# adityaX1412/Experiment-YOLO

Hardware: AMD Instinct MI355X
Metric: images/sec (train) DEAL-YOLO-N 640x640 bs=64/GPU (higher is better)
Workload: dtype f16; 1 GPU; DEAL-YOLO-N (yolov8n-ASF-P2P2.yaml) train step 640x640, per-GPU batch 64, fwd+TAL/WIOU+NWD/DFL/BCE loss+bwd+SGD+EMA, BASELINE.json configs[1]; loss_mode=wiou+nwd, settle_steps=18, capture_retries=0, global_batch=64, parallelism=dp1, hipgraph=True

## Files before the change

experiment-yolo_amd/csrc/conv_wgrad.hip:

```cpp
#include <cstdio>
#include "common.h"
#include "dealyolo_hip.h"

typedef short short4v __attribute__((ext_vector_type(4)));
typedef unsigned int u32x4 __attribute__((ext_vector_type(4)));

struct WgArgs {
  const f16* x;
  const f16* dy;
  float* slabs;
  int ldx, lddy;
  int N, H, W, Ho, Wo;
  int cin_p, cout_p;
  int cin_r8, cout_r8;
  int nci_chunks;
  int tiles_x, tiles_y, ntiles;
  long npix;
  const f16* raw;
  f16* draw;
  const float* coef;
  const double* acc;
  float* dgamma;
  float* dbeta;
  int ldraw, cout;
  float count;
  DySegs xs;
  int dy_csplit;
  unsigned dy_plane;
  const f16* wt;
  f16* dx;
  int lddx, dx_acc;
  int dg_mt, dg_rows;
  DySegs dxs;
};

static __device__ __forceinline__ half8 tr_frag(const char* base0, const char* base1) {
  union {
    short4v s[2];
    half8 h;
  } u;
  u.s[0] = __builtin_amdgcn_ds_read_tr16_b64_v4i16((LDS_AS short4v*)(base0));
  u.s[1] = __builtin_amdgcn_ds_read_tr16_b64_v4i16((LDS_AS short4v*)(base1));
  return u.h;
}

static constexpr __host__ __device__ int wg_th(int ks, int stride, int nci, int mtc) {
  if (ks == 1) return (nci + mtc <= 4) ? 8 : 4;
  if (stride == 1) return (nci * mtc <= 1) ? 16 : ((nci + mtc <= 4) ? 8 : 4);
  return (nci * mtc <= 1) ? 8 : ((nci + mtc <= 4) ? 4 : 2);
}

template <int KS, int STRIDE, int NCI, int MTC, int BNF>
__global__ __launch_bounds__(256, (BNF & 8) ? 3 : ((KS == 3 && NCI * MTC >= 16) ? 1 : 2)) void conv_wgrad_kernel(const WgArgs a) {
  constexpr bool FLAT = (KS == 1);
  constexpr bool DG = (BNF & 4) != 0;
  constexpr bool NOX = (BNF & 8) != 0;
  static_assert(!NOX || DG, "the form without X exists for the fused input gradient only");
  constexpr bool BN1 = ((BNF & 3) == 1 || (BNF & 3) == 3);
  constexpr bool XSEG = ((BNF & 3) == 3);
  static_assert(!DG || (KS == 1 && BN1), "the fused input gradient exists for the 1x1 BatchNorm forms");
  constexpr int TAPS = KS * KS;
  constexpr int NCOL = NCI * TAPS;
  constexpr int CPW = (NCOL + 3) / 4;
  constexpr int TH = wg_th(KS, STRIDE, NCI, MTC), TW = 32;
  constexpr int HWX = FLAT ? TH * TW : (TW - 1) * STRIDE + KS;
  constexpr int HHX = FLAT ? 1 : (TH - 1) * STRIDE + KS;
  constexpr int PAD = KS / 2;
  constexpr int CIN_C = 16 * NCI, COUT_C = 16 * MTC;
  constexpr int PSX = (STRIDE == 2) ? CIN_C * 2 + 16 : (((CIN_C / 2 + 7) / 16) * 16 + 8) * 4;
  constexpr int PSY = (((COUT_C / 2 + 7) / 16) * 16 + 8) * 4;
  constexpr int XBYTES = NOX ? 0 : HHX * HWX * PSX, YBYTES = TH * TW * PSY;
  __shared__ __attribute__((aligned(16))) char smem[XBYTES + YBYTES];
  char* const sx = smem;
  char* const sy = smem + XBYTES;
  __shared__ __attribute__((aligned(16))) float sbn[BN1 ? 4 * COUT_C : (BNF == 2 ? 256 * 8 : 4)];
  float bsum[8] = {0.f, 0.f, 0.f, 0.f, 0.f, 0.f, 0.f, 0.f};
  (void)bsum;
  constexpr int DKS = MTC == 4 ? 2 : (MTC == 3 ? 3 : 1), DCPK = (MTC & 1) ? 16 : 32;
  constexpr int DNT = TH / 2;
  constexpr int DNC = 4 * NCI;
  constexpr int DXROW = CIN_C * 2 + 16;
  constexpr int DPPR = CIN_C / 8;
  constexpr int DPIXPASS = 64 / DPPR > 16 ? 16 : 64 / DPPR;
  constexpr int DNPASS = (16 + DPIXPASS - 1) / DPIXPASS;
  __shared__ __attribute__((aligned(16))) char sdx[DG ? 4 * 16 * DXROW : 16];

  const int tid = threadIdx.x, wave = tid >> 6, lane = tid & 63, p = lane & 15, q = lane >> 4;
  const int qq = p >> 2, pp = p & 3;
  const int co_chunk = blockIdx.y / a.nci_chunks, ci_chunk = blockIdx.y - co_chunk * a.nci_chunks;
  const int ci0 = ci_chunk * CIN_C, co0 = co_chunk * COUT_C;

  f32x4 acc[NOX ? 1 : MTC][NOX ? 1 : CPW];
  if (!NOX) {
#pragma unroll
    for (int m = 0; m < MTC; ++m)
#pragma unroll
      for (int c = 0; c < CPW; ++c) acc[NOX ? 0 : m][NOX ? 0 : c] = (f32x4){0.f, 0.f, 0.f, 0.f};
  }
  (void)acc;

  constexpr int NGX = HHX * HWX * (CIN_C / 8), NGY = TH * TW * (COUT_C / 8);
  constexpr int NPX = NOX ? 1 : (NGX + 255) / 256, NPY = (NGY + 255) / 256;
  uint4 pfx[NPX], pfy[NPY];
  uint4 pfr[BN1 ? NPY : 1];
  unsigned roff[BN1 ? NPY : 1];
  int ncur = 0, nnext = 0;
  (void)ncur; (void)nnext;
  unsigned vnext = 0, vcur = 0, ornext = 0, orcur = 0;
  (void)pfr; (void)roff; (void)vnext; (void)vcur; (void)ornext; (void)orcur;
  constexpr unsigned NEVER = 0x80000000u;
  constexpr int CPGX = CIN_C / 8, CPGY = COUT_C / 8;
  unsigned xoff[NPX], yoff[NPY];
  (void)pfx; (void)xoff;
#pragma unroll
  for (int i = 0; i < NPX; ++i) {
    const int id = tid + i * 256;
    const int pixel = id / CPGX, part = id - pixel * CPGX;
    const bool ok = !NOX && id < NGX && ci0 + part * 8 < a.cin_r8;
    const int hy = FLAT ? 0 : pixel / HWX, hx = FLAT ? pixel : pixel - hy * HWX;
    xoff[i] = ok ? (unsigned)(((hy * a.W + hx) * a.ldx + ci0 + part * 8) * 2) : NEVER;
  }
  constexpr bool XIN = XSEG && !NOX;
  const char* xb[XIN ? NPX : 1];
  int xl[XIN ? NPX : 1];
  unsigned xup = 0;
  bool any_up = false;
  if (XIN)
    for (int k = 0; k < a.xs.nseg; ++k) any_up = any_up || (a.xs.acc[k] & 2);
  (void)xb; (void)xl; (void)xup; (void)any_up;
  if (XIN) {
#pragma unroll
    for (int i = 0; i < NPX; ++i) {
      const int id = tid + i * 256;
      const int part = id % CPGX, ch = ci0 + part * 8;
      int sg = 0;
      while (sg + 1 < a.xs.nseg && ch >= a.xs.c_end[sg]) ++sg;
      const int cb = sg ? a.xs.c_end[sg - 1] : 0;
      const bool ok = id < NGX && ch < a.cin_r8;
      xb[XIN ? i : 0] = ok ? reinterpret_cast<const char*>(a.xs.ptr[sg]) + (ch - cb) * 2 : nullptr;
      xl[XIN ? i : 0] = a.xs.ld[sg] * 2;
      if (ok && (a.xs.acc[sg] & 2)) xup |= 1u << i;
    }
  }
#pragma unroll
  for (int i = 0; i < NPY; ++i) {
    const int id = tid + i * 256;
    const int pixel = id / CPGY, part = id - pixel * CPGY;
    const bool ok = id < NGY && co0 + part * 8 < a.cout_r8;
    const int ty = FLAT ? 0 : pixel / TW, tx = FLAT ? pixel : pixel - ty * TW;
    yoff[i] = ok ? (unsigned)(((ty * a.Wo + tx) * a.lddy + co0 + part * 8) * 2) : NEVER;
    if (FLAT && BN1 && a.dy_csplit && ok) {
      const int ch = co0 + part * 8;
      yoff[i] = (unsigned)((tx * a.lddy + (ch < a.dy_csplit ? ch : ch - a.dy_csplit)) * 2) + (ch < a.dy_csplit ? 0u : a.dy_plane);
    }
    if (BN1) roff[i] = ok ? (unsigned)(((ty * a.Wo + tx) * a.ldraw + co0 + part * 8) * 2) : NEVER;
  }
  if (BN1) {
    for (int c = tid; c < COUT_C; c += 256) {
      const int ch = co0 + c;
      float sc = 0.f, sh = 0.f, kb = 0.f, kc = 0.f;
      if (ch < a.cout) {
        double s1 = 0.0, s2 = 0.0;
#pragma unroll
        for (int k = 0; k < DY_BN_COPIES; ++k) {
          s1 += a.acc[(size_t)(k * 2 + 0) * a.cout + ch];
          s2 += a.acc[(size_t)(k * 2 + 1) * a.cout + ch];
        }
        const float mg = (float)(s1 / a.count), mgx = (float)(s2 / a.count);
        sc = a.coef[ch];
        sh = a.coef[a.cout + ch];
        const float mean = a.coef[2 * a.cout + ch], inv = a.coef[3 * a.cout + ch];
        kb = sc * inv * mgx;
        kc = sc * mg - kb * mean;
        if (!NOX && blockIdx.x == 0 && ci_chunk == 0) {
          if (a.dbeta) a.dbeta[ch] = (float)s1;
          if (a.dgamma) a.dgamma[ch] = (float)s2;
        }
      }
      sbn[c] = sc;
      sbn[COUT_C + c] = sh;
      sbn[2 * COUT_C + c] = kb;
      sbn[3 * COUT_C + c] = kc;
    }
    __syncthreads();
  }
  half8 wf[DG ? DKS : 1][DG ? NCI : 1];
  unsigned dboff[DG ? DKS : 1];
  char* dxb = nullptr;
  unsigned dxld2 = 0;
  bool dxacc = false, dxadd = false;
  const int dpix = lane / DPPR, dpiece = lane - dpix * DPPR;
  (void)wf; (void)dboff; (void)dxb; (void)dxld2; (void)dxacc; (void)dxadd; (void)dpix; (void)dpiece;
  if (DG) {
#pragma unroll
    for (int k = 0; k < DKS; ++k) {
      dboff[DG ? k : 0] = (unsigned)((k * DCPK + ((q * 8) & (DCPK - 1))) * 2);
#pragma unroll
      for (int j = 0; j < NCI; ++j) {
        const int ch = ci0 + (p >> 2) * DNC + 4 * j + (p & 3);
        const int gw = 16 * a.dg_mt, g = ch / gw, rem = ch - g * gw;
        const int row = g * gw + ((rem % (4 * a.dg_mt)) >> 2) * 16 + (rem / (4 * a.dg_mt)) * 4 + (rem & 3);
        const int grow = (g * DKS + k) * gw + (row - g * gw);
        half8 v;
#pragma unroll
        for (int e = 0; e < 8; ++e) v[e] = (f16)0.f;
        if (row < a.dg_rows) v = *reinterpret_cast<const half8*>(a.wt + ((size_t)grow * 32 + q * 8));
        wf[DG ? k : 0][DG ? j : 0] = v;
      }
    }
    const int chn = ci0 + dpiece * 8;
    if (lane < DPIXPASS * DPPR && chn < a.cin_r8) {
      if (XSEG) {
        int sg = 0;
        while (sg + 1 < a.dxs.nseg && chn >= a.dxs.c_end[sg]) ++sg;
        const int cb = sg ? a.dxs.c_end[sg - 1] : 0;
        dxb = reinterpret_cast<char*>(const_cast<void*>(a.dxs.ptr[sg])) + (chn - cb) * 2;
        dxld2 = (unsigned)a.dxs.ld[sg] * 2u;
        dxacc = a.dxs.acc[sg] != 0;
      } else {
        dxb = reinterpret_cast<char*>(a.dx) + chn * 2;
        dxld2 = (unsigned)a.lddx * 2u;
        dxacc = a.dx_acc != 0;
      }
    }
    if (XSEG) {
      for (int k = 0; k < a.dxs.nseg; ++k) dxadd = dxadd || a.dxs.acc[k] != 0;
    } else {
      dxadd = a.dx_acc != 0;
    }
  }
  union DU4 { uint4 u; half2_ h[4]; };
  DU4 dold[DG ? DNT : 1][DG ? DNPASS : 1];
  (void)dold;
  auto ld16 = [](__amdgpu_buffer_rsrc_t r, unsigned off) {
    const auto v = __builtin_amdgcn_raw_buffer_load_b128(r, (int)off, 0, 0);
    return *reinterpret_cast<const uint4*>(&v);
  };
  auto prefetch = [&](int tile) {
    if (FLAT) {
      const auto rx = __builtin_amdgcn_make_buffer_rsrc(const_cast<f16*>(a.x), 0, (int)((unsigned)a.npix * (unsigned)a.ldx * 2u), 0x00020000);
      const auto ry = __builtin_amdgcn_make_buffer_rsrc(const_cast<f16*>(a.dy), 0, (int)((unsigned)a.npix * (unsigned)a.lddy * 2u + (a.dy_csplit ? a.dy_plane : 0u)), 0x00020000);
      const unsigned ox = (unsigned)tile * (TH * TW) * a.ldx * 2u, oy = (unsigned)tile * (TH * TW) * a.lddy * 2u;
      if (NOX) {
      } else if (XIN) {
        const long p0 = (long)tile * (TH * TW);
        int n0 = 0, y0 = 0, x0 = 0;
        if (any_up) {
          const int hw = a.H * a.W, g0 = (int)p0;
          n0 = g0 / hw;
          const int r0 = g0 - n0 * hw;
          y0 = r0 / a.W;
          x0 = r0 - y0 * a.W;
        }
        const float invW = 1.0f / (float)a.W, invH = 1.0f / (float)a.H;
#pragma unroll
        for (int i = 0; i < NPX; ++i) {
          const int lp = (tid + i * 256) / CPGX;
          long gp = p0 + lp;
          const bool inside = gp < a.npix;
          if ((xup >> i) & 1u) {
            const int xx = x0 + lp, dy_ = (int)(((float)xx + 0.5f) * invW), x = xx - dy_ * a.W;
            const int yt = y0 + dy_, dn = (int)(((float)yt + 0.5f) * invH), y = yt - dn * a.H;
            gp = ((long)(n0 + dn) * (a.H >> 1) + (y >> 1)) * (a.W >> 1) + (x >> 1);
          }
          const char* src = xb[XIN ? i : 0];
          pfx[i] = (src && inside) ? *reinterpret_cast<const uint4*>(src + gp * xl[XIN ? i : 0]) : make_uint4(0, 0, 0, 0);
        }
      } else {
#pragma unroll
        for (int i = 0; i < NPX; ++i) pfx[i] = ld16(rx, xoff[i] + ox);
      }
#pragma unroll
      for (int i = 0; i < NPY; ++i) pfy[i] = ld16(ry, yoff[i] + oy);
      if (BN1) {
        const unsigned nbytes = (unsigned)a.npix * (unsigned)a.ldraw * 2u;
        const auto rr = __builtin_amdgcn_make_buffer_rsrc(const_cast<f16*>(a.raw), 0, (int)nbytes, 0x00020000);
        ornext = (unsigned)tile * (TH * TW) * a.ldraw * 2u;
        vnext = 0;
#pragma unroll
        for (int i = 0; i < NPY; ++i) {
          const unsigned off = roff[i] + ornext;
          pfr[i] = ld16(rr, off);
          vnext |= (roff[i] != NEVER && off < nbytes) ? (1u << i) : 0u;
        }
      }
    } else {
      const int bx = tile % a.tiles_x;
      const int t2 = tile / a.tiles_x;
      const int n = t2 / a.tiles_y;
      const int oy0 = (t2 % a.tiles_y) * TH, ox0 = bx * TW;
      const int iy0 = oy0 * STRIDE - PAD, ix0 = ox0 * STRIDE - PAD;
      const auto rx = __builtin_amdgcn_make_buffer_rsrc(const_cast<f16*>(a.x) + (size_t)n * a.H * a.W * a.ldx, 0, a.H * a.W * a.ldx * 2, 0x00020000);
      const auto ry = __builtin_amdgcn_make_buffer_rsrc(const_cast<f16*>(a.dy) + (size_t)n * a.Ho * a.Wo * a.lddy, 0, a.Ho * a.Wo * a.lddy * 2, 0x00020000);
      const unsigned ox = (unsigned)((iy0 * a.W + ix0) * a.ldx * 2), oy = (unsigned)((oy0 * a.Wo + ox0) * a.lddy * 2);
      if (ix0 >= 0 && ix0 + HWX <= a.W) {
#pragma unroll
        for (int i = 0; i < NPX; ++i) pfx[i] = ld16(rx, xoff[i] + ox);
      } else {
#pragma unroll
        for (int i = 0; i < NPX; ++i) {
          const int hx = ((tid + i * 256) / CPGX) % HWX;
          pfx[i] = ld16(rx, (unsigned)(ix0 + hx) < (unsigned)a.W ? xoff[i] + ox : NEVER);
        }
      }
      if (ox0 + TW <= a.Wo) {
#pragma unroll
        for (int i = 0; i < NPY; ++i) pfy[i] = ld16(ry, yoff[i] + oy);
      } else {
#pragma unroll
        for (int i = 0; i < NPY; ++i) {
          const int tx = ((tid + i * 256) / CPGY) % TW;
          pfy[i] = ld16(ry, ox0 + tx < a.Wo ? yoff[i] + oy : NEVER);
        }
      }
      if (BN1) {
        const unsigned nbytes = (unsigned)(a.Ho * a.Wo * a.ldraw * 2);
        const auto rr = __builtin_amdgcn_make_buffer_rsrc(const_cast<f16*>(a.raw) + (size_t)n * a.Ho * a.Wo * a.ldraw, 0, (int)nbytes, 0x00020000);
        ornext = (unsigned)((oy0 * a.Wo + ox0) * a.ldraw * 2);
        vnext = 0;
        const bool xfull = ox0 + TW <= a.Wo;
#pragma unroll
        for (int i = 0; i < NPY; ++i) {
          unsigned off = roff[i] == NEVER ? NEVER : roff[i] + ornext;
          if (!xfull) {
            const int tx = ((tid + i * 256) / CPGY) % TW;
            off = ox0 + tx < a.Wo ? off : NEVER;
          }
          pfr[i] = ld16(rr, off);
          vnext |= off < nbytes ? (1u << i) : 0u;
        }
        nnext = n;
      }
    }
  };


  int tile = (!FLAT && !(gridDim.x & 7)) ? (int)(blockIdx.x & 7) * (int)(gridDim.x >> 3) + (int)(blockIdx.x >> 3) : (int)blockIdx.x;
  if (tile < a.ntiles) prefetch(tile);
  for (; tile < a.ntiles; tile += gridDim.x) {
    __syncthreads();
#pragma unroll
    for (int i = 0; i < NPX; ++i) {
      const int id = tid + i * 256;
      if (!NOX && id < NGX) *reinterpret_cast<uint4*>(sx + (id / (CIN_C / 8)) * PSX + (id % (CIN_C / 8)) * 16) = pfx[i];
    }
    if (BN1) {
      vcur = vnext; orcur = ornext; ncur = nnext;
      const unsigned nbytes = FLAT ? (unsigned)a.npix * (unsigned)a.ldraw * 2u : (unsigned)(a.Ho * a.Wo * a.ldraw * 2);
      const auto rd = __builtin_amdgcn_make_buffer_rsrc(FLAT ? a.draw : a.draw + (size_t)ncur * a.Ho * a.Wo * a.ldraw, 0, (int)nbytes, 0x00020000);
#pragma unroll
      for (int i = 0; i < NPY; ++i) {
        const int id = tid + i * 256;
        const int part = id % CPGY;
        const bool valid = (vcur >> i) & 1u;
        const float* cf = sbn + part * 8;
        union { half8 h; uint4 u; u32x4 v; } o;
        o.h = bn_bwd_apply8<DY_ACT_SILU>(*reinterpret_cast<const half8*>(&pfy[i]), *reinterpret_cast<const half8*>(&pfr[i]), cf,
                                         cf + COUT_C, cf + 2 * COUT_C, cf + 3 * COUT_C);
        if (!valid) o.u = make_uint4(0, 0, 0, 0);
        if (id < NGY) *reinterpret_cast<uint4*>(sy + (id / (COUT_C / 8)) * PSY + (id % (COUT_C / 8)) * 16) = o.u;
        if (!DG && ci_chunk == 0 && a.draw) __builtin_amdgcn_raw_buffer_store_b128(o.v, rd, (int)(valid ? roff[i] + orcur : NEVER), 0, 0);
      }
    } else {
#pragma unroll
      for (int i = 0; i < NPY; ++i) {
        const int id = tid + i * 256;
        if (id < NGY) *reinterpret_cast<uint4*>(sy + (id / (COUT_C / 8)) * PSY + (id % (COUT_C / 8)) * 16) = pfy[i];
        if (BNF == 2 && id < NGY) {
          const half8 v = *reinterpret_cast<const half8*>(&pfy[i]);
#pragma unroll
          for (int j = 0; j < 8; ++j) bsum[j] += (float)v[j];
        }
      }
    }
    __syncthreads();
    const long dpix0 = (long)tile * (TH * TW) + wave * (16 * DNT);
    (void)dpix0;
    if (DG && dxadd) {
#pragma unroll
      for (int t = 0; t < DNT; ++t)
#pragma unroll
        for (int ps = 0; ps < DNPASS; ++ps) {
          const int rowi = ps * DPIXPASS + dpix;
          const long gp = dpix0 + t * 16 + rowi;
          const bool ok = dxb && dxacc && rowi < 16 && gp < a.npix;
          dold[DG ? t : 0][DG ? ps : 0].u = ok ? *reinterpret_cast<const uint4*>(dxb + (size_t)gp * dxld2) : make_uint4(0, 0, 0, 0);
        }
      __builtin_amdgcn_sched_barrier(0);
    }
    if (tile + (int)gridDim.x < a.ntiles) prefetch(tile + gridDim.x);
    if constexpr (!NOX) {
    const int kpix = 4 * q + qq;
    half8 af[2][MTC], bf[2];
    auto load_a = [&](int buf, int r) {
#pragma unroll
      for (int m = 0; m < MTC; ++m) {
        const char* b0 = sy + (r * TW + kpix) * PSY + (m * 16 + 4 * pp) * 2;
        af[buf][m] = tr_frag(b0, b0 + 16 * PSY);
      }
    };
    auto load_b = [&](int buf, int r, int c) {
      const int col = wave + 4 * c;
      if (col < NCOL) {
        const int cit = col / TAPS, tap = col - cit * TAPS;
        const int dy = tap / KS, dx = tap - dy * KS;
        const char* b0;
        int step;
        if (FLAT) {
          b0 = sx + (r * TW + kpix) * PSX + (cit * 16 + 4 * pp) * 2;
          step = 16 * PSX;
        } else {
          b0 = sx + ((r * STRIDE + dy) * HWX + kpix * STRIDE + dx) * PSX + (cit * 16 + 4 * pp) * 2;
          step = 16 * STRIDE * PSX;
        }
        bf[buf] = tr_frag(b0, b0 + step);
      }
    };
    load_a(0, 0);
    load_b(0, 0, 0);
#pragma unroll
    for (int r = 0; r < TH; ++r) {
      if (r + 1 < TH) load_a((r + 1) & 1, r + 1);
#pragma unroll
      for (int c = 0; c < CPW; ++c) {
        const int lin = r * CPW + c;
        if (c + 1 < CPW) load_b((lin + 1) & 1, r, c + 1);
        else if (r + 1 < TH) load_b((lin + 1) & 1, r + 1, 0);
        __builtin_amdgcn_sched_barrier(0);
        if (wave + 4 * c < NCOL) {
#pragma unroll
          for (int m = 0; m < MTC; ++m)
            acc[NOX ? 0 : m][NOX ? 0 : c] = __builtin_amdgcn_mfma_f32_16x16x32_f16(af[r & 1][m], bf[lin & 1], acc[NOX ? 0 : m][NOX ? 0 : c], 0, 0, 0);
        }
        __builtin_amdgcn_sched_barrier(0);
      }
    }
    }
    if (DG) {
      half8 db[DNT][DKS];
#pragma unroll
      for (int t = 0; t < DNT; ++t)
#pragma unroll
        for (int k = 0; k < DKS; ++k)
          db[t][k] = *reinterpret_cast<const half8*>(sy + ((wave * DNT + t) * 16 + p) * PSY + dboff[DG ? k : 0]);
      f32x4 dacc[NCI][DNT];
#pragma unroll
      for (int j = 0; j < NCI; ++j)
#pragma unroll
        for (int t = 0; t < DNT; ++t) dacc[j][t] = (f32x4){0.f, 0.f, 0.f, 0.f};
#pragma unroll
      for (int k = 0; k < DKS; ++k)
#pragma unroll
        for (int j = 0; j < NCI; ++j)
#pragma unroll
          for (int t = 0; t < DNT; ++t)
            dacc[j][t] = __builtin_amdgcn_mfma_f32_16x16x32_f16(wf[DG ? k : 0][DG ? j : 0], db[t][k], dacc[j][t], 0, 0, 0);
      typedef uint2 __attribute__((may_alias)) uint2_a;
      typedef uint4 __attribute__((may_alias)) uint4_a;
      char* const xs = sdx + wave * (16 * DXROW);
      char* const xw = xs + p * DXROW + q * (DNC * 2);
      const int rrow = dpix < 16 ? dpix : 15;
      auto lds_order = []() {
        __builtin_amdgcn_fence(__ATOMIC_RELEASE, "wavefront", "local");
        __builtin_amdgcn_wave_barrier();
        __builtin_amdgcn_fence(__ATOMIC_ACQUIRE, "wavefront", "local");
      };
#pragma unroll
      for (int t = 0; t < DNT; ++t) {
        union { half2_ h[DNC / 2]; uint2 u2[DNC / 4]; } hv;
#pragma unroll
        for (int j = 0; j < NCI; ++j) {
          const f32x2 lo = {dacc[j][t][0], dacc[j][t][1]}, hi = {dacc[j][t][2], dacc[j][t][3]};
          hv.h[j * 2] = __builtin_convertvector(lo, half2_);
          hv.h[j * 2 + 1] = __builtin_convertvector(hi, half2_);
        }
        lds_order();
#pragma unroll
        for (int j = 0; j < NCI; ++j) reinterpret_cast<uint2_a*>(xw)[j] = hv.u2[j];
        lds_order();
#pragma unroll
        for (int ps = 0; ps < DNPASS; ++ps) {
          const int rowi = ps * DPIXPASS + dpix;
          const int rr = ps * DPIXPASS + rrow < 16 ? ps * DPIXPASS + rrow : 15;
          DU4 v;
          v.u = *reinterpret_cast<const uint4_a*>(xs + rr * DXROW + dpiece * 16);
          const long gp = dpix0 + t * 16 + rowi;
          if (dxadd) {
#pragma unroll
            for (int k = 0; k < 4; ++k)
              v.h[k] = __builtin_convertvector(__builtin_convertvector(v.h[k], f32x2) + __builtin_convertvector(dold[DG ? t : 0][DG ? ps : 0].h[k], f32x2), half2_);
          }
          if (dxb && rowi < 16 && gp < a.npix) *reinterpret_cast<uint4*>(dxb + (size_t)gp * dxld2) = v.u;
        }
      }
    }
  }

  if (BNF == 2 && ci_chunk == 0) {
    __syncthreads();
#pragma unroll
    for (int j = 0; j < 8; ++j) sbn[tid * 8 + j] = bsum[j];
    __syncthreads();
    if (tid < COUT_C && co0 + tid < a.cout) {
      const int part = tid >> 3, j = tid & 7;
      float t = 0.f;
      for (int k = part; k < 256; k += CPGY) t += sbn[k * 8 + j];
      unsafeAtomicAdd(const_cast<double*>(a.acc) + (size_t)(blockIdx.x % DY_BN_COPIES) * a.cout + co0 + tid, (double)t);
    }
  }
  if constexpr (NOX) return;
  float* slab = a.slabs + (size_t)blockIdx.x * TAPS * a.cout_p * a.cin_p;
#pragma unroll
  for (int c = 0; c < CPW; ++c) {
    const int col = wave + 4 * c;
    if (col < NCOL) {
      const int cit = col / TAPS, tap = col - cit * TAPS;
#pragma unroll
      for (int m = 0; m < MTC; ++m)
#pragma unroll
        for (int r = 0; r < 4; ++r) {
          const int co = co0 + m * 16 + q * 4 + r, ci = ci0 + cit * 16 + p;
          slab[((size_t)tap * a.cout_p + co) * a.cin_p + ci] = acc[NOX ? 0 : m][NOX ? 0 : c][r];
        }
    }
  }
}

static __device__ __forceinline__ void wgrad_reduce_block(int block, const float* slabs, int nslabs, float* dw, int cout, int cin,
                                                          int taps, int cout_p, int cin_p, int accumulate,
                                                          int ld_taps, int ld_cphys, int ld_cin) {
  const int lane = threadIdx.x & 63, grp = threadIdx.x >> 6;
  const long S = (long)taps * cout_p * cin_p;
  const long o = (long)block * 64 + lane;
  float s0 = 0.f, s1 = 0.f, s2 = 0.f, s3 = 0.f;
  if (o < S) {
    const float* p = slabs + o;
    int k = grp;
    for (; k + 12 < nslabs; k += 16) {
      s0 += p[(long)k * S];
      s1 += p[(long)(k + 4) * S];
      s2 += p[(long)(k + 8) * S];
      s3 += p[(long)(k + 12) * S];
    }
    for (; k < nslabs; k += 4) s0 += p[(long)k * S];
  }
  __shared__ float red[4][64];
  red[grp][lane] = (s0 + s1) + (s2 + s3);
  __syncthreads();
  if (grp == 0 && o < S) {
    const float tot = (red[0][lane] + red[1][lane]) + (red[2][lane] + red[3][lane]);
    const int ci = (int)(o % cin_p);
    const long t = o / cin_p;
    const int co = (int)(t % cout_p), tap = (int)(t / cout_p);
    if (ld_taps) {
      const int n = ci / ld_cphys, ch = ci - n * ld_cphys;
      if (co < cout && n < ld_taps && ch < ld_cin) {
        float* d = dw + ((long)co * ld_cin + ch) * ld_taps + n;
        *d = accumulate ? *d + tot : tot;
      }
    } else if (co < cout && ci < cin) {
      float* d = dw + ((long)co * cin + ci) * taps + tap;
      *d = accumulate ? *d + tot : tot;
    }
  }
}

__global__ __launch_bounds__(256) void wgrad_reduce_kernel(const float* slabs, int nslabs, float* dw, int cout, int cin,
                                                           int taps, int cout_p, int cin_p, int accumulate,
                                                           int ld_taps, int ld_cphys, int ld_cin) {
  wgrad_reduce_block(blockIdx.x, slabs, nslabs, dw, cout, cin, taps, cout_p, cin_p, accumulate, ld_taps, ld_cphys, ld_cin);
}

struct WgReduceDesc {
  const float* slabs;
  float* dw;
  int nslabs, cout, cin, taps, cout_p, cin_p, accumulate, ld_taps, ld_cphys, ld_cin;
  int first_block, bias_c;
  const double* bias_acc;
  float* dbias;
};
__global__ __launch_bounds__(256) void wgrad_reduce_batched_kernel(const WgReduceDesc* descs, int n) {
  int lo = 0, hi = n - 1;
  while (lo < hi) {
    const int mid = (lo + hi + 1) >> 1;
    if (descs[mid].first_block <= (int)blockIdx.x) lo = mid;
    else hi = mid - 1;
  }
  const WgReduceDesc d = descs[lo];
  if (d.bias_c > 0 && (int)blockIdx.x == d.first_block && (int)threadIdx.x < d.bias_c) {
    double t = 0.0;
#pragma unroll
    for (int k = 0; k < DY_BN_COPIES; ++k) t += d.bias_acc[(size_t)k * d.bias_c + threadIdx.x];
    d.dbias[threadIdx.x] = (float)t;
  }
  wgrad_reduce_block(blockIdx.x - d.first_block, d.slabs, d.nslabs, d.dw, d.cout, d.cin, d.taps, d.cout_p, d.cin_p, d.accumulate,
                     d.ld_taps, d.ld_cphys, d.ld_cin);
}
extern "C" int dy_wgrad_reduce_desc_bytes(void) { return (int)sizeof(WgReduceDesc); }
static void wgrad_geometry(int cin, int cout, int ks, int stride, int* cin_p, int* cout_p, int* nci, int* mtc, long npix_out = 0);
extern "C" int dy_wgrad_reduce_desc_fill(void* desc, const float* slabs, int nslabs, float* dw, int cin, int cout, int ks, int stride,
                                         int accumulate, int ld_taps, int ld_cphys, int ld_cin, int first_block) {
  if (!desc || !slabs || !dw || nslabs < 1) return DY_ERR_ARG;
  int cp, op, nci, mtc;
  const int cin_eff = ld_taps ? ld_taps * ld_cphys : cin;
  wgrad_geometry(cin_eff, cout, ld_taps ? 1 : ks, ld_taps ? 1 : stride, &cp, &op, &nci, &mtc);
  const int taps = ld_taps ? 1 : ks * ks;
  WgReduceDesc* d = reinterpret_cast<WgReduceDesc*>(desc);
  *d = WgReduceDesc{slabs, dw, nslabs, cout, cin_eff, taps, op, cp, accumulate, ld_taps, ld_cphys, ld_cin, first_block, 0, nullptr, nullptr};
  return cdiv(taps * op * cp, 64);
}
extern "C" int dy_wgrad_reduce_desc_bias(void* desc, const double* bias_acc, float* dbias, int c) {
  if (!desc || !bias_acc || !dbias || c < 1 || c > 256) return DY_ERR_ARG;
  WgReduceDesc* d = reinterpret_cast<WgReduceDesc*>(desc);
  d->bias_acc = bias_acc; d->dbias = dbias; d->bias_c = c;
  return DY_OK;
}
extern "C" int dy_wgrad_reduce_batched(const void* descs_device, int n, int total_blocks, hipStream_t stream) {
  if (n <= 0 || total_blocks <= 0 || !descs_device) return DY_ERR_ARG;
  hipLaunchKernelGGL(wgrad_reduce_batched_kernel, dim3(total_blocks), dim3(256), 0, stream, (const WgReduceDesc*)descs_device, n);
  DY_CHECK_LAUNCH();
  return DY_OK;
}

template <int KS, int STRIDE, int NCI, int MTC>
static int launch_wgrad(const WgArgs& a, int gx, int gy, hipStream_t s) {
  if (a.wt) {
    if constexpr (KS == 1) {
      if (!a.raw || gy != a.nci_chunks) return DY_ERR_ARG;
      if (!a.x) {
        if (a.dxs.nseg > 0) hipLaunchKernelGGL((conv_wgrad_kernel<KS, STRIDE, NCI, MTC, 15>), dim3(gx, gy), dim3(256), 0, s, a);
        else hipLaunchKernelGGL((conv_wgrad_kernel<KS, STRIDE, NCI, MTC, 13>), dim3(gx, gy), dim3(256), 0, s, a);
      } else if (a.xs.nseg > 0) hipLaunchKernelGGL((conv_wgrad_kernel<KS, STRIDE, NCI, MTC, 7>), dim3(gx, gy), dim3(256), 0, s, a);
      else hipLaunchKernelGGL((conv_wgrad_kernel<KS, STRIDE, NCI, MTC, 5>), dim3(gx, gy), dim3(256), 0, s, a);
    } else return DY_ERR_ARG;
  } else if (a.raw && a.xs.nseg > 0) {
    if constexpr (KS == 1) hipLaunchKernelGGL((conv_wgrad_kernel<KS, STRIDE, NCI, MTC, 3>), dim3(gx, gy), dim3(256), 0, s, a);
    else return DY_ERR_ARG;
  } else if (a.raw) hipLaunchKernelGGL((conv_wgrad_kernel<KS, STRIDE, NCI, MTC, 1>), dim3(gx, gy), dim3(256), 0, s, a);
  else if (a.acc && MTC != 3) hipLaunchKernelGGL((conv_wgrad_kernel<KS, STRIDE, NCI, MTC, 2>), dim3(gx, gy), dim3(256), 0, s, a);
  else if (a.acc) return DY_ERR_ARG;
  else hipLaunchKernelGGL((conv_wgrad_kernel<KS, STRIDE, NCI, MTC, 0>), dim3(gx, gy), dim3(256), 0, s, a);
  DY_CHECK_LAUNCH();
  return DY_OK;
}
template <int KS, int STRIDE>
static int dispatch_wgrad(int nci, int mtc, const WgArgs& a, int gx, int gy, hipStream_t s) {
#define DY_CASE(I, M) \
  if (nci == I && mtc == M) return launch_wgrad<KS, STRIDE, I, M>(a, gx, gy, s);
  DY_CASE(1, 1) DY_CASE(1, 2) DY_CASE(1, 4)
  DY_CASE(2, 1) DY_CASE(2, 2) DY_CASE(2, 4)
  if (!(KS == 3 && STRIDE == 2)) { DY_CASE(4, 1) DY_CASE(4, 2) DY_CASE(4, 4) }
  if (KS == 1) {
    DY_CASE(3, 1) DY_CASE(3, 2) DY_CASE(3, 4) DY_CASE(1, 3) DY_CASE(2, 3) DY_CASE(4, 3) DY_CASE(3, 3)
  }
#undef DY_CASE
  return DY_ERR_ARG;
}

static int wgrad_per_cu(int ks, int nci, int mtc) {
  static const int light = getenv("DY_WGRAD_LIGHT_WGS") ? atoi(getenv("DY_WGRAD_LIGHT_WGS")) : 2;
  if (ks == 3 && nci * mtc >= 16) return 1;
  return nci * mtc <= 2 ? light : 2;
}
static long wgrad_columns(int ks, int nci, int mtc, int cp, int op) {
  const int gy = (cp / (16 * nci)) * (op / (16 * mtc));
  const int per_cu = wgrad_per_cu(ks, nci, mtc);
  int gx = (256 * per_cu) / gy;
  return gx < 32 ? 32 : gx;
}
static void wgrad_geometry(int cin, int cout, int ks, int stride, int* cin_p, int* cout_p, int* nci, int* mtc, long npix_out) {
  *cin_p = (cin + 15) / 16 * 16;
  *cout_p = (cout + 15) / 16 * 16;
  const int cit = *cin_p / 16, cot = *cout_p / 16;
  const int cap = (ks == 3 && stride == 2) ? 2 : 4;
  *nci = (cit % 4 == 0 && cap >= 4) ? 4 : ((ks == 1 && cit % 3 == 0) ? 3 : (cit % 2 == 0 ? 2 : 1));
  *mtc = cot % 4 == 0 ? 4 : ((ks == 1 && cot % 3 == 0) ? 3 : (cot % 2 == 0 ? 2 : 1));
  static const bool split = !(getenv("DY_WGRAD_SPLIT") && atoi(getenv("DY_WGRAD_SPLIT")) == 0);
  static const double f = getenv("DY_WGRAD_SPLIT_F") ? atof(getenv("DY_WGRAD_SPLIT_F")) : 2.0;
  if (!split || npix_out <= 0) return;
  const double wbytes = (double)ks * ks * *cin_p * *cout_p * 4.0;
  const double act = (double)npix_out * (*cin_p * stride * stride + *cout_p) * 2.0;
  while (2.0 * wgrad_columns(ks, *nci, *mtc, *cin_p, *cout_p) * wbytes > f * act) {
    if (*mtc % 2 == 0 && *mtc >= *nci) *mtc /= 2;
    else if (*nci % 2 == 0) *nci /= 2;
    else if (*mtc % 2 == 0) *mtc /= 2;
    else break;
  }
}

extern "C" int dy_wgrad_workspace(int n, int h, int w, int cin, int cout, int ks, int stride, int* nslabs,
                                  long* slab_elems) {
  int cp, op, nci, mtc;
  const int pad = ks / 2, Ho = (h + 2 * pad - ks) / stride + 1, Wo = (w + 2 * pad - ks) / stride + 1;
  wgrad_geometry(cin, cout, ks, stride, &cp, &op, &nci, &mtc, (long)n * Ho * Wo);
  const int th = wg_th(ks, stride, nci, mtc);
  int ntiles;
  if (ks == 1) ntiles = (int)(((long)n * Ho * Wo + th * 32 - 1) / (th * 32));
  else ntiles = cdiv(Wo, 32) * cdiv(Ho, th) * n;
  *slab_elems = (long)ks * ks * cp * op;
  const int gy = (cp / (16 * nci)) * (op / (16 * mtc));
  const int per_cu = wgrad_per_cu(ks, nci, mtc);
  int gx = (256 * per_cu) / gy;
  if (gx < 32) gx = 32;
  static const int tpb = getenv("DY_WGRAD_TPB") ? atoi(getenv("DY_WGRAD_TPB")) : 1;
  if (tpb > 1 && gx > ntiles / tpb) gx = ntiles / tpb > 32 ? ntiles / tpb : (ntiles < 32 ? ntiles : 32);
  if (gx > ntiles) gx = ntiles;
  if (gx < 1) gx = 1;
  *nslabs = gx;
  return DY_OK;
}

struct WgBnHost {
  const void* raw; void* draw; const float* coef; const double* acc; float* dgamma; float* dbeta; int ldraw; float count;
  const DySegs* xs = nullptr;
  int dy_csplit = 0;
  unsigned dy_plane = 0;
  const void* wt = nullptr; void* dx = nullptr; int lddx = 0, dx_acc = 0; const DySegs* dxs = nullptr;
  bool dgrad_only = false;
};
static int conv_wgrad_impl(const void* x, int ldx, const void* dy, int lddy, float* slabs, float* dw, int n, int h, int w,
                           int cin, int cout, int ks, int stride, int accumulate, int ld_taps, int ld_cphys, int ld_cin,
                           hipStream_t stream, const WgBnHost* bn = nullptr);

extern "C" int dy_wgrad_kernel_name(int cin, int cout, int ks, int stride, char* out, int cap) {
  if (!out || cap < 8) return DY_ERR_ARG;
  int cp, op, nci, mtc;
  wgrad_geometry(cin, cout, ks, stride, &cp, &op, &nci, &mtc);
  snprintf(out, cap, "conv_wgrad_kernel<%d, %d, %d, %d, 0>", ks, stride, nci, mtc);
  return DY_OK;
}

extern "C" int dy_wgrad_kernel_name_at(int n, int h, int w, int cin, int cout, int ks, int stride, char* out, int cap) {
  if (!out || cap < 8) return DY_ERR_ARG;
  int cp, op, nci, mtc;
  wgrad_geometry(cin, cout, ks, stride, &cp, &op, &nci, &mtc,
                 (long)n * ((h + 2 * (ks / 2) - ks) / stride + 1) * ((w + 2 * (ks / 2) - ks) / stride + 1));
  snprintf(out, cap, "conv_wgrad_kernel<%d, %d, %d, %d, 0>", ks, stride, nci, mtc);
  return DY_OK;
}

extern "C" int dy_conv_wgrad(const void* x, int ldx, const void* dy, int lddy, float* slabs, float* dw, int n, int h,
                             int w, int cin, int cout, int ks, int stride, int accumulate, hipStream_t stream) {
  return conv_wgrad_impl(x, ldx, dy, lddy, slabs, dw, n, h, w, cin, cout, ks, stride, accumulate, 0, 0, 0, stream);
}
extern "C" int dy_conv_wgrad_ld(const void* x, int ldx, const void* dy, int lddy, float* slabs, float* dw, int n, int h,
                                int w, int cout, int ld_cin, int ld_taps, int ld_cphys, int accumulate, hipStream_t stream) {
  return conv_wgrad_impl(x, ldx, dy, lddy, slabs, dw, n, h, w, ld_taps * ld_cphys, cout, 1, 1, accumulate, ld_taps, ld_cphys,
                         ld_cin, stream);
}

extern "C" int dy_conv_wgrad_bn(const void* x, int ldx, const void* dy, int lddy, const void* raw, int ldraw, void* draw,
                                const float* coef, const double* acc, float* dgamma, float* dbeta, float count, float* slabs,
                                float* dw, int n, int h, int w, int cin, int cout, int ks, int stride, int accumulate,
                                hipStream_t stream) {
  if (!raw || !coef || !acc || (ldraw & 7) || ((uintptr_t)raw & 15) || ((uintptr_t)draw & 15) || (cout & 15)) return DY_ERR_ARG;
  const WgBnHost bn{raw, draw, coef, acc, dgamma, dbeta, ldraw, count};
  return conv_wgrad_impl(x, ldx, dy, lddy, slabs, dw, n, h, w, cin, cout, ks, stride, accumulate, 0, 0, 0, stream, &bn);
}
extern "C" int dy_conv_wgrad_bias(const void* x, int ldx, const void* dy, int lddy, double* bias_acc, float* slabs, float* dw, int n,
                                  int h, int w, int cin, int cout, int ks, int stride, int accumulate, hipStream_t stream) {
  if (!bias_acc) return DY_ERR_ARG;
  const WgBnHost bn{nullptr, nullptr, nullptr, bias_acc, nullptr, nullptr, 0, 1.f};
  return conv_wgrad_impl(x, ldx, dy, lddy, slabs, dw, n, h, w, cin, cout, ks, stride, accumulate, 0, 0, 0, stream, &bn);
}
extern "C" int dy_conv1x1_wgrad_bn_segs(const DySegs* xs, const void* dy, int lddy, const void* raw, int ldraw, void* draw, const float* coef,
                                        const double* acc, float* dgamma, float* dbeta, float count, float* slabs, float* dw, int n, int h,
                                        int w, int cin, int cout, int accumulate, hipStream_t stream) {
  if (!raw || !coef || !acc || (ldraw & 7) || ((uintptr_t)raw & 15) || ((uintptr_t)draw & 15) || (cout & 15)) return DY_ERR_ARG;
  if (!xs || xs->nseg < 1 || xs->nseg > DY_MAX_SEGS || xs->c_end[xs->nseg - 1] != cin) return DY_ERR_ARG;
  for (int k = 0; k < xs->nseg; ++k)
    if ((xs->c_end[k] & 7) || (xs->ld[k] & 7) || !xs->ptr[k] || ((uintptr_t)xs->ptr[k] & 15) || xs->c_end[k] <= (k ? xs->c_end[k - 1] : 0) ||
        ((xs->acc[k] & 2) && ((h | w) & 1))) return DY_ERR_ARG;
  WgBnHost bn{raw, draw, coef, acc, dgamma, dbeta, ldraw, count};
  bn.xs = xs;
  return conv_wgrad_impl(xs->ptr[0], 8, dy, lddy, slabs, dw, n, h, w, cin, cout, 1, 1, accumulate, 0, 0, 0, stream, &bn);
}
extern "C" int dy_conv1x1_wgrad_bn_planes(const DySegs* xs, const void* x, int ldx, const void* dy, const void* dy2, int lddy, int csplit,
                                          const void* raw, int ldraw, void* draw, const float* coef, const double* acc, float* dgamma,
                                          float* dbeta, float count, float* slabs, float* dw, int n, int h, int w, int cin, int cout,
                                          int accumulate, hipStream_t stream) {
  if (!raw || !coef || !acc || (ldraw & 7) || ((uintptr_t)raw & 15) || ((uintptr_t)draw & 15) || (cout & 15)) return DY_ERR_ARG;
  if (!dy || !dy2 || (csplit & 7) || csplit <= 0 || csplit >= cout || ((uintptr_t)dy2 & 15)) return DY_ERR_ARG;
  const long plane = (const char*)dy2 - (const char*)dy;
  if (plane < (long)n * h * w * lddy * 2 || plane + (double)n * h * w * lddy * 2.0 >= 2147483648.0) return DY_ERR_ARG;
  if (xs) {
    if (xs->nseg < 1 || xs->nseg > DY_MAX_SEGS || xs->c_end[xs->nseg - 1] != cin) return DY_ERR_ARG;
    for (int k = 0; k < xs->nseg; ++k)
      if ((xs->c_end[k] & 7) || (xs->ld[k] & 7) || !xs->ptr[k] || ((uintptr_t)xs->ptr[k] & 15) || xs->c_end[k] <= (k ? xs->c_end[k - 1] : 0) ||
          ((xs->acc[k] & 2) && ((h | w) & 1))) return DY_ERR_ARG;
  }
  WgBnHost bn{raw, draw, coef, acc, dgamma, dbeta, ldraw, count};
  bn.xs = xs;
  bn.dy_csplit = csplit; bn.dy_plane = (unsigned)plane;
  return conv_wgrad_impl(xs ? xs->ptr[0] : x, xs ? 8 : ldx, dy, lddy, slabs, dw, n, h, w, cin, cout, 1, 1, accumulate, 0, 0, 0, stream, &bn);
}

struct WgDgPlan { int ok, nci, mtc, dg_mt, dg_rows; };
static WgDgPlan wgrad_dgrad_plan(int n, int h, int w, int cin, int cout) {
  WgDgPlan r{};
  if (n < 1 || h < 1 || w < 1 || cin < 8 || (cin & 7) || cout < 16 || (cout & 15) || cout > 64) return r;
  int cp, op, nci, mtc;
  wgrad_geometry(cin, cout, 1, 1, &cp, &op, &nci, &mtc, (long)n * h * w);
  if (16 * mtc != op) return r;
  int gcin, gcout, cc, nch, mt, ng, kst, pe;
  if (dy_conv_geometry(cout, cin, 1, 1, &gcin, &gcout, &cc, &nch, &mt, &ng, &kst, &pe) != DY_OK) return r;
  const int dks = mtc == 4 ? 2 : (mtc == 3 ? 3 : 1), dcpk = (mtc & 1) ? 16 : 32;
  if (gcin != cout || nch * kst != dks || (cc < 32 ? cc : 32) != dcpk || gcout < cp) return r;
  r.ok = 1; r.nci = nci; r.mtc = mtc; r.dg_mt = mt; r.dg_rows = gcout;
  return r;
}
extern "C" int dy_conv1x1_wgrad_dgrad_supported(int n, int h, int w, int cin, int cout) { return wgrad_dgrad_plan(n, h, w, cin, cout).ok; }
extern "C" int dy_wgrad_dgrad_kernel_name(int n, int h, int w, int cin, int cout, int segs, char* out, int cap) {
  const WgDgPlan pl = wgrad_dgrad_plan(n, h, w, cin, cout);
  if (!out || cap < 8 || !pl.ok) return DY_ERR_ARG;
  snprintf(out, cap, "conv_wgrad_kernel<1, 1, %d, %d, %d>", pl.nci, pl.mtc, segs ? 7 : 5);
  return DY_OK;
}
static bool dgrad_segs_valid(const DySegs* xs, const DySegs* dxs) {
  if (!xs || !dxs || dxs->nseg != xs->nseg) return false;
  for (int k = 0; k < dxs->nseg; ++k) {
    const int cb = k ? dxs->c_end[k - 1] : 0;
    if (dxs->c_end[k] != xs->c_end[k] || (dxs->ld[k] & 7) || dxs->ld[k] < dxs->c_end[k] - cb || !dxs->ptr[k] || ((uintptr_t)dxs->ptr[k] & 15) ||
        (dxs->acc[k] & ~1)) return false;
  }
  return true;
}
static bool segs_in_valid(const DySegs* xs, int cin, int h, int w) {
  if (!xs || xs->nseg < 1 || xs->nseg > DY_MAX_SEGS || xs->c_end[xs->nseg - 1] != cin) return false;
  for (int k = 0; k < xs->nseg; ++k)
    if ((xs->c_end[k] & 7) || (xs->ld[k] & 7) || !xs->ptr[k] || ((uintptr_t)xs->ptr[k] & 15) || xs->c_end[k] <= (k ? xs->c_end[k - 1] : 0) ||
        ((xs->acc[k] & 2) && ((h | w) & 1))) return false;
  return true;
}
static int dgrad_only_columns(int ntiles, int gy) {
  int gx = (256 * 3) / (gy > 0 ? gy : 1);
  if (gx < 32) gx = 32;
  if (gx > ntiles) gx = ntiles;
  return gx < 1 ? 1 : gx;
}
extern "C" int dy_conv1x1_dgrad_bn_supported(int n, int h, int w, int cin, int cout) { return wgrad_dgrad_plan(n, h, w, cin, cout).ok; }
extern "C" int dy_dgrad_only_kernel_name(int n, int h, int w, int cin, int cout, int segs, char* out, int cap) {
  const WgDgPlan pl = wgrad_dgrad_plan(n, h, w, cin, cout);
  if (!out || cap < 8 || !pl.ok) return DY_ERR_ARG;
  snprintf(out, cap, "conv_wgrad_kernel<1, 1, %d, %d, %d>", pl.nci, pl.mtc, segs ? 15 : 13);
  return DY_OK;
}
extern "C" int dy_conv1x1_dgrad_bn(const void* dy, const void* dy2, int lddy, int csplit, const void* raw, int ldraw, const float* coef,
                                   const double* acc, float count, const void* w_packed_t, void* dx, int lddx, int dx_accumulate,
                                   const DySegs* dxs, int n, int h, int w, int cin, int cout, hipStream_t stream) {
  if (!dy || !raw || !coef || !acc || (ldraw & 7) || ((uintptr_t)raw & 15)) return DY_ERR_ARG;
  if (!w_packed_t || ((uintptr_t)w_packed_t & 15) || !wgrad_dgrad_plan(n, h, w, cin, cout).ok) return DY_ERR_ARG;
  long plane = 0;
  if (dy2) {
    if ((csplit & 7) || csplit <= 0 || csplit >= cout || ((uintptr_t)dy2 & 15)) return DY_ERR_ARG;
    plane = (const char*)dy2 - (const char*)dy;
    if (plane < (long)n * h * w * lddy * 2 || plane + (double)n * h * w * lddy * 2.0 >= 2147483648.0) return DY_ERR_ARG;
  } else if (csplit) {
    return DY_ERR_ARG;
  }
  if (dxs) {
    if (dxs->nseg < 1 || dxs->nseg > DY_MAX_SEGS || dxs->c_end[dxs->nseg - 1] != cin) return DY_ERR_ARG;
    for (int k = 0; k < dxs->nseg; ++k) {
      const int cb = k ? dxs->c_end[k - 1] : 0;
      if ((dxs->c_end[k] & 7) || dxs->c_end[k] <= cb || (dxs->ld[k] & 7) || dxs->ld[k] < dxs->c_end[k] - cb || !dxs->ptr[k] ||
          ((uintptr_t)dxs->ptr[k] & 15) || (dxs->acc[k] & ~1)) return DY_ERR_ARG;
    }
  } else if (!dx || ((uintptr_t)dx & 15) || (lddx & 7) || lddx < cin || (double)n * h * w * lddx * 2.0 >= 2147483648.0) {
    return DY_ERR_ARG;
  }
  WgBnHost bn{raw, nullptr, coef, acc, nullptr, nullptr, ldraw, count};
  bn.dy_csplit = dy2 ? csplit : 0; bn.dy_plane = (unsigned)plane;
  bn.wt = w_packed_t; bn.dxs = dxs; bn.dx = dxs ? nullptr : dx; bn.lddx = lddx; bn.dx_acc = dx_accumulate != 0;
  bn.dgrad_only = true;
  return conv_wgrad_impl(nullptr, 8, dy, lddy, nullptr, nullptr, n, h, w, cin, cout, 1, 1, 0, 0, 0, 0, stream, &bn);
}
extern "C" int dy_conv1x1_wgrad_dgrad_bn(const void* x, int ldx, const void* dy, int lddy, const void* raw, int ldraw, const float* coef,
                                         const double* acc, float* dgamma, float* dbeta, float count, float* slabs, float* dw,
                                         const void* w_packed_t, void* dx, int lddx, int dx_accumulate, int n, int h, int w, int cin,
                                         int cout, int accumulate, hipStream_t stream) {
  if (!raw || !coef || !acc || (ldraw & 7) || ((uintptr_t)raw & 15)) return DY_ERR_ARG;
  if (!w_packed_t || ((uintptr_t)w_packed_t & 15) || !dx || ((uintptr_t)dx & 15) || (lddx & 7) || lddx < cin) return DY_ERR_ARG;
  if (!wgrad_dgrad_plan(n, h, w, cin, cout).ok || (double)n * h * w * lddx * 2.0 >= 2147483648.0) return DY_ERR_ARG;
  WgBnHost bn{raw, nullptr, coef, acc, dgamma, dbeta, ldraw, count};
  bn.wt = w_packed_t; bn.dx = dx; bn.lddx = lddx; bn.dx_acc = dx_accumulate != 0;
  return conv_wgrad_impl(x, ldx, dy, lddy, slabs, dw, n, h, w, cin, cout, 1, 1, accumulate, 0, 0, 0, stream, &bn);
}
extern "C" int dy_conv1x1_wgrad_dgrad_bn_segs(const DySegs* xs, const void* dy, int lddy, const void* raw, int ldraw, const float* coef,
                                              const double* acc, float* dgamma, float* dbeta, float count, float* slabs, float* dw,
                                              const void* w_packed_t, const DySegs* dxs, int n, int h, int w, int cin, int cout,
                                              int accumulate, hipStream_t stream) {
  if (!raw || !coef || !acc || (ldraw & 7) || ((uintptr_t)raw & 15)) return DY_ERR_ARG;
  if (!w_packed_t || ((uintptr_t)w_packed_t & 15) || !segs_in_valid(xs, cin, h, w) || !dgrad_segs_valid(xs, dxs)) return DY_ERR_ARG;
  if (!wgrad_dgrad_plan(n, h, w, cin, cout).ok) return DY_ERR_ARG;
  WgBnHost bn{raw, nullptr, coef, acc, dgamma, dbeta, ldraw, count};
  bn.xs = xs; bn.wt = w_packed_t; bn.dxs = dxs;
  return conv_wgrad_impl(xs->ptr[0], 8, dy, lddy, slabs, dw, n, h, w, cin, cout, 1, 1, accumulate, 0, 0, 0, stream, &bn);
}
extern "C" int dy_conv1x1_wgrad_dgrad_bn_planes(const DySegs* xs, const void* x, int ldx, const void* dy, const void* dy2, int lddy, int csplit,
                                                const void* raw, int ldraw, const float* coef, const double* acc, float* dgamma,
                                                float* dbeta, float count, float* slabs, float* dw, const void* w_packed_t, void* dx,
                                                int lddx, int dx_accumulate, const DySegs* dxs, int n, int h, int w, int cin, int cout,
                                                int accumulate, hipStream_t stream) {
  if (!raw || !coef || !acc || (ldraw & 7) || ((uintptr_t)raw & 15)) return DY_ERR_ARG;
  if (!dy || !dy2 || (csplit & 7) || csplit <= 0 || csplit >= cout || ((uintptr_t)dy2 & 15)) return DY_ERR_ARG;
  const long plane = (const char*)dy2 - (const char*)dy;
  if (plane < (long)n * h * w * lddy * 2 || plane + (double)n * h * w * lddy * 2.0 >= 2147483648.0) return DY_ERR_ARG;
  if (!w_packed_t || ((uintptr_t)w_packed_t & 15) || !wgrad_dgrad_plan(n, h, w, cin, cout).ok) return DY_ERR_ARG;
  if (xs) {
    if (!segs_in_valid(xs, cin, h, w) || !dgrad_segs_valid(xs, dxs)) return DY_ERR_ARG;
  } else if (dxs || !dx || ((uintptr_t)dx & 15) || (lddx & 7) || lddx < cin || (double)n * h * w * lddx * 2.0 >= 2147483648.0) {
    return DY_ERR_ARG;
  }
  WgBnHost bn{raw, nullptr, coef, acc, dgamma, dbeta, ldraw, count};
  bn.xs = xs; bn.dy_csplit = csplit; bn.dy_plane = (unsigned)plane;
  bn.wt = w_packed_t; bn.dxs = xs ? dxs : nullptr; bn.dx = xs ? nullptr : dx; bn.lddx = lddx; bn.dx_acc = dx_accumulate != 0;
  return conv_wgrad_impl(xs ? xs->ptr[0] : x, xs ? 8 : ldx, dy, lddy, slabs, dw, n, h, w, cin, cout, 1, 1, accumulate, 0, 0, 0, stream, &bn);
}
extern "C" int dy_conv_wgrad_ld_bn(const void* x, int ldx, const void* dy, int lddy, const void* raw, int ldraw, void* draw,
                                   const float* coef, const double* acc, float* dgamma, float* dbeta, float count, float* slabs,
                                   float* dw, int n, int h, int w, int cout, int ld_cin, int ld_taps, int ld_cphys, int accumulate,
                                   hipStream_t stream) {
  if (!raw || !coef || !acc || (ldraw & 7) || ((uintptr_t)raw & 15) || ((uintptr_t)draw & 15) || (cout & 15)) return DY_ERR_ARG;
  const WgBnHost bn{raw, draw, coef, acc, dgamma, dbeta, ldraw, count};
  return conv_wgrad_impl(x, ldx, dy, lddy, slabs, dw, n, h, w, ld_taps * ld_cphys, cout, 1, 1, accumulate, ld_taps, ld_cphys, ld_cin,
                         stream, &bn);
}

static int conv_wgrad_impl(const void* x, int ldx, const void* dy, int lddy, float* slabs, float* dw, int n, int h, int w,
                           int cin, int cout, int ks, int stride, int accumulate, int ld_taps, int ld_cphys, int ld_cin,
                           hipStream_t stream, const WgBnHost* bn) {
  if (!(ks == 1 || ks == 3) || !(stride == 1 || stride == 2) || (ks == 1 && stride != 1)) return DY_ERR_ARG;
  if ((ldx & 7) || (lddy & 7) || ((uintptr_t)x & 15) || ((uintptr_t)dy & 15)) return DY_ERR_ALIGN;
  const bool dgrad_only = bn && bn->dgrad_only;
  if (dgrad_only != (x == nullptr) || (dgrad_only && (!bn->wt || slabs || dw))) return DY_ERR_ARG;
  if ((ks == 1 ? (double)n : 1.0) * h * w * (ldx > lddy ? ldx : lddy) * 2.0 >= 2147483648.0) return DY_ERR_ARG;
  int cp, op, nci, mtc;
  wgrad_geometry(cin, cout, ks, stride, &cp, &op, &nci, &mtc,
                 (long)n * ((h + 2 * (ks / 2) - ks) / stride + 1) * ((w + 2 * (ks / 2) - ks) / stride + 1));
  WgArgs a{};
  a.x = (const f16*)x; a.dy = (const f16*)dy; a.slabs = slabs; a.ldx = ldx; a.lddy = lddy;
  a.N = n; a.H = h; a.W = w;
  const int pad = ks / 2;
  a.Ho = (h + 2 * pad - ks) / stride + 1;
  a.Wo = (w + 2 * pad - ks) / stride + 1;
  a.cin_p = cp; a.cout_p = op;
  a.cin_r8 = (cin + 7) / 8 * 8; a.cout_r8 = (cout + 7) / 8 * 8;
  if (bn) {
    if ((ks == 1 ? (double)n : 1.0) * a.Ho * a.Wo * bn->ldraw * 2.0 >= 2147483648.0) return DY_ERR_ARG;
    a.raw = (const f16*)bn->raw; a.draw = (f16*)bn->draw; a.coef = bn->coef; a.acc = bn->acc;
    a.dgamma = bn->dgamma; a.dbeta = bn->dbeta; a.ldraw = bn->ldraw; a.count = bn->count;
    a.cout = bn->raw ? cout : (cout + 7) / 8 * 8;
    if (bn->xs) a.xs = *bn->xs;
    a.dy_csplit = bn->dy_csplit; a.dy_plane = bn->dy_plane;
    if (bn->wt) {
      const WgDgPlan pl = wgrad_dgrad_plan(n, h, w, cin, cout);
      if (!pl.ok || pl.nci != nci || pl.mtc != mtc || ks != 1 || ld_taps) return DY_ERR_ARG;
      a.wt = (const f16*)bn->wt; a.dx = (f16*)bn->dx; a.lddx = bn->lddx; a.dx_acc = bn->dx_acc;
      a.dg_mt = pl.dg_mt; a.dg_rows = pl.dg_rows;
      if (bn->dxs) a.dxs = *bn->dxs;
    }
  }
  a.nci_chunks = cp / (16 * nci);
  const int nco_chunks = op / (16 * mtc);
  const int th = wg_th(ks, stride, nci, mtc);
  if (ks == 1) {
    a.npix = (long)n * a.Ho * a.Wo;
    a.ntiles = (int)((a.npix + th * 32 - 1) / (th * 32));
  } else {
    a.tiles_x = cdiv(a.Wo, 32);
    a.tiles_y = cdiv(a.Ho, th);
    a.ntiles = a.tiles_x * a.tiles_y * n;
  }
  int nslabs;
  long slab_elems;
  dy_wgrad_workspace(n, h, w, cin, cout, ks, stride, &nslabs, &slab_elems);
  const int gy = a.nci_chunks * nco_chunks;
  if (dgrad_only) nslabs = dgrad_only_columns(a.ntiles, gy);
  int rc;
  if (ks == 1) rc = dispatch_wgrad<1, 1>(nci, mtc, a, nslabs, gy, stream);
  else if (stride == 1) rc = dispatch_wgrad<3, 1>(nci, mtc, a, nslabs, gy, stream);
  else rc = dispatch_wgrad<3, 2>(nci, mtc, a, nslabs, gy, stream);
  if (rc != DY_OK) return rc;
  if (!dw) return DY_OK;
  const int total = ks * ks * op * cp;
  hipLaunchKernelGGL(wgrad_reduce_kernel, dim3(cdiv(total, 64)), dim3(256), 0, stream, slabs, nslabs, dw, cout, cin,
                     ks * ks, op, cp, accumulate, ld_taps, ld_cphys, ld_cin);
  DY_CHECK_LAUNCH();
  return DY_OK;
}
```

experiment-yolo_amd/csrc/stem.hip:

```cpp
#include "common.h"
#include "dealyolo_hip.h"

#define STEM_CO 16
#define STEM_TH 8
#define STEM_TW 32
#define STEM_IH (2 * STEM_TH + 1)
#define STEM_IW (2 * STEM_TW + 1)
#define STEM_IP 68

struct StemArgs {
  const float* img;
  const float* w;
  f16* raw;
  double* acc;
  const f16* dy;
  const float* coef;
  float* dgamma;
  float* dbeta;
  float* slabs;
  int N, H, W, Ho, Wo, ldraw, lddy, tiles_x, tiles_y, ntiles;
  float mul, count;
  const float* bias;
  int silu;
};

static __device__ __forceinline__ void stem_stage(const StemArgs& a, f16 (*s_in)[STEM_IH][STEM_IP], int n, int oy0, int ox0) {
  const int wave = threadIdx.x >> 6, lane = threadIdx.x & 63;
  const int iy0 = 2 * oy0 - 1, ix0 = 2 * ox0 - 1;
  const float* img = a.img + (size_t)n * 3 * a.H * a.W;
#pragma unroll 1
  for (int r0 = 0; r0 < 3 * STEM_IH; r0 += 4 * 4) {
    float v[4], ve[4];
#pragma unroll
    for (int u = 0; u < 4; ++u) {
      const int r = r0 + u * 4 + wave;
      const int c = (r >= STEM_IH) + (r >= 2 * STEM_IH), y = r - c * STEM_IH, iy = iy0 + y, ix = ix0 + lane;
      const bool rowok = r < 3 * STEM_IH && (unsigned)iy < (unsigned)a.H;
      const float* row = img + ((size_t)c * a.H + (rowok ? iy : 0)) * a.W;
      v[u] = (rowok && (unsigned)ix < (unsigned)a.W) ? row[ix] : 0.f;
      ve[u] = (rowok && lane == 0 && ix0 + 64 < a.W) ? row[ix0 + 64] : 0.f;
    }
#pragma unroll
    for (int u = 0; u < 4; ++u) {
      const int r = r0 + u * 4 + wave;
      if (r < 3 * STEM_IH) {
        const int c = (r >= STEM_IH) + (r >= 2 * STEM_IH), y = r - c * STEM_IH;
        s_in[c][y][lane] = (f16)(v[u] * a.mul);
        if (lane == 0) s_in[c][y][64] = (f16)(ve[u] * a.mul);
      }
    }
  }
}

typedef _Float16 half4_ __attribute__((ext_vector_type(4)));
typedef uint2 __attribute__((aligned(4))) uint2_a4;

template <bool INFER>
__global__ __launch_bounds__(256) void stem_fwd_kernel(StemArgs a) {
  __shared__ __attribute__((aligned(16))) f16 s_in[3][STEM_IH][STEM_IP];
  __shared__ float s_red[4][2][STEM_CO];
  const int tid = threadIdx.x, wave = tid >> 6, lane = tid & 63, p = lane & 15, q = lane >> 4;
  half4_ af[3];
  int goff[3];
#pragma unroll
  for (int ks = 0; ks < 3; ++ks) {
    const int g = ks * 4 + q, gc = g < 9 ? g : 8, c = gc / 3, ky = gc - c * 3;
    goff[ks] = (c * STEM_IH + ky) * STEM_IP;
#pragma unroll
    for (int kx = 0; kx < 4; ++kx) af[ks][kx] = (g < 9 && kx < 3) ? (f16)a.w[p * 27 + c * 9 + ky * 3 + kx] : (f16)0.f;
  }
  f32x4 s1 = {0.f, 0.f, 0.f, 0.f}, s2 = s1;
  f32x4 b4 = {0.f, 0.f, 0.f, 0.f};
  if (INFER && a.bias) b4 = *reinterpret_cast<const f32x4*>(a.bias + q * 4);
  const f16* s_flat = &s_in[0][0][0];
  for (int e = tid; e < 3 * STEM_IH * (STEM_IP - STEM_IW); e += 256)
    (&s_in[0][0][0])[(e / (STEM_IP - STEM_IW)) * STEM_IP + STEM_IW + e % (STEM_IP - STEM_IW)] = (f16)0.f;
  for (int tile = blockIdx.x; tile < a.ntiles; tile += gridDim.x) {
    const int bx = tile % a.tiles_x, t2 = tile / a.tiles_x;
    const int by = t2 % a.tiles_y, n = t2 / a.tiles_y;
    const int oy0 = by * STEM_TH, ox0 = bx * STEM_TW;
    __syncthreads();
    stem_stage(a, s_in, n, oy0, ox0);
    __syncthreads();
#pragma unroll
    for (int nt = 0; nt < 4; ++nt) {
      const int ty = wave * 2 + (nt >> 1), px = (nt & 1) * 16 + p;
      f32x4 acc = {0.f, 0.f, 0.f, 0.f};
#pragma unroll
      for (int ks = 0; ks < 3; ++ks) {
        union { uint2 u; half4_ h; } bf;
        const uint2_a4* src = reinterpret_cast<const uint2_a4*>(s_flat + goff[ks] + (2 * ty) * STEM_IP + 2 * px);
        bf.u.x = src->x;
        bf.u.y = src->y;
        acc = __builtin_amdgcn_mfma_f32_16x16x16f16(af[ks], bf.h, acc, 0, 0, 0);
      }
      const int oy = oy0 + ty, ox = ox0 + px;
      if (oy < a.Ho && ox < a.Wo) {
        union { half4_ h; uint2 u; } o;
        if (INFER) {
          acc += b4;
          if (a.silu) acc = (f32x4){silu_f(acc[0]), silu_f(acc[1]), silu_f(acc[2]), silu_f(acc[3])};
        }
        o.h = __builtin_convertvector(acc, half4_);
        *reinterpret_cast<uint2*>(a.raw + (((size_t)n * a.Ho + oy) * a.Wo + ox) * a.ldraw + q * 4) = o.u;
        if (!INFER) {
          s1 += acc;
          s2 += acc * acc;
        }
      }
    }
  }
  if (INFER) return;
#pragma unroll
  for (int r = 0; r < 4; ++r) {
    const float r1 = quad16_sum(s1[r]), r2 = quad16_sum(s2[r]);
    if (p == 0) {
      s_red[wave][0][q * 4 + r] = r1;
      s_red[wave][1][q * 4 + r] = r2;
    }
  }
  __syncthreads();
  if (tid < 2 * STEM_CO) {
    const int which = tid / STEM_CO, ch = tid - which * STEM_CO;
    const float s = (s_red[0][which][ch] + s_red[1][which][ch]) + (s_red[2][which][ch] + s_red[3][which][ch]);
    unsafeAtomicAdd(&a.acc[((size_t)(blockIdx.x % DY_BN_COPIES) * 2 + which) * STEM_CO + ch], (double)s);
  }
}

#define STEM_DP (STEM_TH * STEM_TW + 8)
__global__ __launch_bounds__(256) void stem_wgrad_bn_kernel(StemArgs a) {
  __shared__ __attribute__((aligned(16))) f16 s_in[3][STEM_IH][STEM_IP];
  __shared__ __attribute__((aligned(16))) f16 s_d[STEM_CO][STEM_DP];
  __shared__ float s_bn[4][STEM_CO];
  __shared__ float s_acc[4][2][16][16];
  const int tid = threadIdx.x, wave = tid >> 6, lane = tid & 63, p = lane & 15, q = lane >> 4;
  if (tid < STEM_CO) {
    double t1 = 0.0, t2 = 0.0;
#pragma unroll
    for (int k = 0; k < DY_BN_COPIES; ++k) {
      t1 += a.acc[(size_t)(k * 2 + 0) * STEM_CO + tid];
      t2 += a.acc[(size_t)(k * 2 + 1) * STEM_CO + tid];
    }
    const float mg = (float)(t1 / a.count), mgx = (float)(t2 / a.count);
    const float sc = a.coef[tid], sh = a.coef[STEM_CO + tid], mean = a.coef[2 * STEM_CO + tid], inv = a.coef[3 * STEM_CO + tid];
    const float kb = sc * inv * mgx;
    s_bn[0][tid] = sc;
    s_bn[1][tid] = sh;
    s_bn[2][tid] = kb;
    s_bn[3][tid] = sc * mg - kb * mean;
    if (blockIdx.x == 0) {
      if (a.dbeta) a.dbeta[tid] = (float)t1;
      if (a.dgamma) a.dgamma[tid] = (float)t2;
    }
  }
  f32x4 acc[2] = {(f32x4){0.f, 0.f, 0.f, 0.f}, (f32x4){0.f, 0.f, 0.f, 0.f}};
  for (int e = tid; e < 3 * STEM_IH * (STEM_IP - STEM_IW); e += 256)
    (&s_in[0][0][0])[(e / (STEM_IP - STEM_IW)) * STEM_IP + STEM_IW + e % (STEM_IP - STEM_IW)] = (f16)0.f;
  int boff[2];
  bool bok[2];
#pragma unroll
  for (int nt = 0; nt < 2; ++nt) {
    const int kk = nt * 16 + p, c = kk / 9, r = kk - c * 9, ky = r / 3, kx = r - ky * 3;
    bok[nt] = kk < 27;
    boff[nt] = bok[nt] ? (c * STEM_IH + ky) * STEM_IP + kx : 0;
  }
  const f16* s_in_flat = &s_in[0][0][0];
  for (int tile = blockIdx.x; tile < a.ntiles; tile += gridDim.x) {
    const int bx = tile % a.tiles_x, t2 = tile / a.tiles_x;
    const int by = t2 % a.tiles_y, n = t2 / a.tiles_y;
    const int oy0 = by * STEM_TH, ox0 = bx * STEM_TW;
    __syncthreads();
    const int ty = tid >> 5, tx = tid & 31, oy = oy0 + ty, ox = ox0 + tx;
    const bool pv = oy < a.Ho && ox < a.Wo;
    const size_t pix = pv ? ((size_t)n * a.Ho + oy) * a.Wo + ox : 0;
    const half8 d0 = *reinterpret_cast<const half8*>(a.dy + pix * a.lddy), d1 = *reinterpret_cast<const half8*>(a.dy + pix * a.lddy + 8);
    const half8 r0 = *reinterpret_cast<const half8*>(a.raw + pix * a.ldraw), r1 = *reinterpret_cast<const half8*>(a.raw + pix * a.ldraw + 8);
    stem_stage(a, s_in, n, oy0, ox0);
    {
      half8 o0 = bn_bwd_apply8<DY_ACT_SILU>(d0, r0, s_bn[0], s_bn[1], s_bn[2], s_bn[3]);
      half8 o1 = bn_bwd_apply8<DY_ACT_SILU>(d1, r1, s_bn[0] + 8, s_bn[1] + 8, s_bn[2] + 8, s_bn[3] + 8);
#pragma unroll
      for (int j = 0; j < 8; ++j) {
        s_d[j][tid] = pv ? o0[j] : (f16)0.f;
        s_d[8 + j][tid] = pv ? o1[j] : (f16)0.f;
      }
    }
    __syncthreads();
#pragma unroll
    for (int ks = 0; ks < 2; ++ks) {
      const int row = wave * 2 + ks, pix0 = row * STEM_TW + q * 8;
      const half8 af = *reinterpret_cast<const half8*>(&s_d[p][pix0]);
      half8 bf[2];
#pragma unroll
      for (int nt = 0; nt < 2; ++nt) {
        const f16* b = s_in_flat + boff[nt] + (2 * row) * STEM_IP + 2 * (q * 8);
#pragma unroll
        for (int j = 0; j < 8; ++j) bf[nt][j] = bok[nt] ? b[2 * j] : (f16)0.f;
      }
      acc[0] = __builtin_amdgcn_mfma_f32_16x16x32_f16(af, bf[0], acc[0], 0, 0, 0);
      acc[1] = __builtin_amdgcn_mfma_f32_16x16x32_f16(af, bf[1], acc[1], 0, 0, 0);
    }
  }
#pragma unroll
  for (int nt = 0; nt < 2; ++nt)
#pragma unroll
    for (int r = 0; r < 4; ++r) s_acc[wave][nt][q * 4 + r][p] = acc[nt][r];
  __syncthreads();
  float* slab = a.slabs + (size_t)blockIdx.x * 9 * 16 * 16;
  for (int e = tid; e < 27 * STEM_CO; e += 256) {
    const int kk = e / STEM_CO, co = e - kk * STEM_CO, c = kk / 9, tap = kk - c * 9, nt = kk >> 4, col = kk & 15;
    const float s = (s_acc[0][nt][co][col] + s_acc[1][nt][co][col]) + (s_acc[2][nt][co][col] + s_acc[3][nt][co][col]);
    slab[((size_t)tap * 16 + co) * 16 + c] = s;
  }
}

static int stem_args(StemArgs& a, int n, int h, int w) {
  if (n < 1 || h < 2 || w < 2) return DY_ERR_ARG;
  a.N = n; a.H = h; a.W = w;
  a.Ho = (h + 2 - 3) / 2 + 1;
  a.Wo = (w + 2 - 3) / 2 + 1;
  a.tiles_x = cdiv(a.Wo, STEM_TW);
  a.tiles_y = cdiv(a.Ho, STEM_TH);
  a.ntiles = a.tiles_x * a.tiles_y * n;
  return DY_OK;
}
static int stem_fwd_grid(int ntiles) { return ntiles < 2048 ? ntiles : 2048; }
extern "C" int dy_stem_grid(int n, int h, int w) {
  StemArgs a{};
  if (stem_args(a, n, h, w) != DY_OK) return DY_ERR_ARG;
  return a.ntiles < 1024 ? a.ntiles : 1024;
}

extern "C" int dy_stem_forward(const float* img_nchw, const float* weight, void* raw, int ldraw, double* acc, int n, int h, int w,
                               float mul, hipStream_t stream) {
  StemArgs a{};
  if (!img_nchw || !weight || !raw || !acc || (ldraw & 7) || ((uintptr_t)raw & 15)) return DY_ERR_ARG;
  if (stem_args(a, n, h, w) != DY_OK) return DY_ERR_ARG;
  a.img = img_nchw; a.w = weight; a.raw = (f16*)raw; a.acc = acc; a.ldraw = ldraw; a.mul = mul;
  hipLaunchKernelGGL(stem_fwd_kernel<false>, dim3(stem_fwd_grid(a.ntiles)), dim3(256), 0, stream, a);
  DY_CHECK_LAUNCH();
  return DY_OK;
}

extern "C" int dy_stem_forward_eval(const float* img_nchw, const float* weight, const float* bias, void* y, int ldy, int n, int h, int w,
                                    float mul, int silu, hipStream_t stream) {
  StemArgs a{};
  if (!img_nchw || !weight || !y || (ldy & 7) || ((uintptr_t)y & 15) || (bias && ((uintptr_t)bias & 15))) return DY_ERR_ARG;
  if (stem_args(a, n, h, w) != DY_OK) return DY_ERR_ARG;
  a.img = img_nchw; a.w = weight; a.raw = (f16*)y; a.ldraw = ldy; a.mul = mul; a.bias = bias; a.silu = silu;
  hipLaunchKernelGGL(stem_fwd_kernel<true>, dim3(stem_fwd_grid(a.ntiles)), dim3(256), 0, stream, a);
  DY_CHECK_LAUNCH();
  return DY_OK;
}

extern "C" int dy_stem_wgrad_bn(const float* img_nchw, const void* dy, int lddy, const void* raw, int ldraw, const float* coef,
                                const double* acc, float* dgamma, float* dbeta, float count, float* slabs, int n, int h, int w,
                                float mul, hipStream_t stream) {
  StemArgs a{};
  if (!img_nchw || !dy || !raw || !coef || !acc || !slabs || (ldraw & 7) || (lddy & 7) || ((uintptr_t)raw & 15) || ((uintptr_t)dy & 15))
    return DY_ERR_ARG;
  if (stem_args(a, n, h, w) != DY_OK) return DY_ERR_ARG;
  a.img = img_nchw; a.dy = (const f16*)dy; a.raw = (f16*)const_cast<void*>(raw); a.coef = coef; a.acc = const_cast<double*>(acc);
  a.dgamma = dgamma; a.dbeta = dbeta; a.slabs = slabs; a.ldraw = ldraw; a.lddy = lddy; a.mul = mul; a.count = count;
  hipLaunchKernelGGL(stem_wgrad_bn_kernel, dim3(dy_stem_grid(n, h, w)), dim3(256), 0, stream, a);
  DY_CHECK_LAUNCH();
  return DY_OK;
}
```

experiment-yolo_amd/ultralytics/hip/__init__.py:

```python
from __future__ import annotations

import ctypes as C
import os
import sys

_FLAG = "DEBUG_CLR_GRAPH_PACKET_CAPTURE"


def _hip_already_up():
    t = sys.modules.get("torch")
    try:
        return bool(t is not None and t.cuda.is_initialized())
    except Exception:
        return False


if os.environ.get(_FLAG) is None and not _hip_already_up():
    os.environ[_FLAG] = "0"
GRAPH_SAFE = os.environ.get(_FLAG) == "0"

_HERE = os.path.dirname(os.path.abspath(__file__))
LIB_PATH = os.environ.get("DY_HIP_LIB") or os.path.normpath(os.path.join(_HERE, "..", "..", "csrc", "libdealyolo_hip.so"))

DY_EPI_STATS, DY_EPI_BIAS, DY_EPI_SILU, DY_EPI_F32OUT, DY_EPI_ACCUM, DY_EPI_STATS_ACC = 1, 2, 4, 8, 16, 32
DY_BN_COPIES = 16
DY_ACT_NONE, DY_ACT_SILU, DY_ACT_LEAKY = 0, 1, 2
_ERR = {-1: "DY_ERR_ARG (unsupported shape/argument)", -2: "DY_ERR_LAUNCH (HIP launch failed)",
        -3: "DY_ERR_ALIGN (pointer/stride alignment)", -4: "DY_ERR_CAPACITY (more items than the kernel's table holds)"}

vp, i32, f32, i64, sz = C.c_void_p, C.c_int, C.c_float, C.c_long, C.c_size_t
ip = C.POINTER(C.c_int)
lp = C.POINTER(C.c_long)


class DyLossArgs(C.Structure):
    _fields_ = [("nl", i32), ("B", i32), ("nc", i32), ("ncp", i32), ("nmax", i32),
                ("box", vp * 4), ("cls", vp * 4), ("dbox", vp * 4), ("dcls", vp * 4),
                ("H", i32 * 4), ("W", i32 * 4), ("stride", f32 * 4),
                ("t_batch_idx", vp), ("t_cls", vp), ("t_boxes", vp), ("n_targets", i32), ("n_targets_dev", vp),
                ("img_w", f32), ("img_h", f32), ("hyp_box", f32), ("hyp_cls", f32), ("hyp_dfl", f32),
                ("use_wiou", i32), ("use_nwd", i32), ("iou_ratio", f32), ("gscale", vp), ("scalars", vp),
                ("workspace", vp), ("dbox_rows_only", i32), ("box_from_input", i32), ("box_in", vp * 4), ("box_in_ld", i32 * 4),
                ("box_w", vp * 4), ("box_b", vp * 4), ("box_in_coef", vp * 4),
                ("box_family", i32), ("box_ltype", i32), ("box_fm", i32), ("box_modifier", i32), ("inner_ratio", f32),
                ("focaler_d", f32), ("focaler_u", f32), ("shape_scale", f32), ("piou_lambda", f32)]


class DySegs(C.Structure):
    _fields_ = [("nseg", i32), ("c_end", i32 * 8), ("ld", i32 * 8), ("acc", i32 * 8), ("ptr", vp * 8)]


SIGNATURES = {
    "dy_abi_version": (i32, []),
    "dy_loss_args_bytes": (i32, []),
    "dy_conv_geometry": (i32, [i32, i32, i32, i32, ip, ip, ip, ip, ip, ip, ip, ip]),
    "dy_pack_weights": (i32, [vp, vp, vp, i32, i32, i32, i32, i32, vp]),
    "dy_pack_desc_bytes": (i32, []),
    "dy_pack_desc_fill": (i32, [vp, vp, vp, vp, i32, i32, i32, i32, i32, i32, i32, i32]),
    "dy_pack_weights_batched": (i32, [vp, i32, i32, vp]),
    "dy_conv_forward": (i32, [vp, i32, vp, vp, vp, i32, vp, i32, i32, i32, i32, i32, i32, i32, i32, i32, i32, i32, ip, vp]),
    "dy_segs_bytes": (i32, []),
    "dy_conv1x1_segs_supported": (i32, [i32, i32, C.POINTER(DySegs)]),
    "dy_conv1x1_forward_segs": (i32, [C.POINTER(DySegs), vp, vp, vp, i32, vp, i32, i32, i32, i32, i32, i32, vp]),
    "dy_conv1x1_input_grad_segs": (i32, [vp, i32, vp, C.POINTER(DySegs), i32, i32, i32, i32, i32, vp]),
    "dy_conv1x1_wgrad_bn_segs": (i32, [C.POINTER(DySegs), vp, i32, vp, i32, vp, vp, vp, vp, vp, f32, vp, vp, i32, i32, i32, i32, i32, i32, vp]),
    "dy_conv_res_supported": (i32, [i32, i32, i32, i32]),
    "dy_conv_forward_res": (i32, [vp, i32, vp, vp, vp, i32, vp, i32, i32, i32, i32, i32, i32, i32, i32, vp]),
    "dy_conv_red_supported": (i32, [i32, i32, i32]),
    "dy_conv_input_grad_red": (i32, [vp, i32, vp, vp, i32, i32, i32, i32, i32, i32, i32, vp, i32, vp, vp, i32, vp]),
    "dy_conv_kernel_name": (i32, [i32, i32, i32, i32, C.c_char_p, i32]),
    "dy_conv1x1_segs_kernel_name": (i32, [i32, i32, C.POINTER(DySegs), C.c_char_p, i32]),
    "dy_conv1x1_kernel_name_live": (i32, [i32, i32, i32, i32, i32, i32, C.POINTER(DySegs), C.POINTER(DySegs), C.c_char_p, i32]),
    "dy_conv_kernel_name_at": (i32, [i32, i32, i32, i32, i32, i32, i32, C.c_char_p, i32]),
    "dy_wgrad_kernel_name": (i32, [i32, i32, i32, i32, C.c_char_p, i32]),
    "dy_wgrad_kernel_name_at": (i32, [i32, i32, i32, i32, i32, i32, i32, C.c_char_p, i32]),
    "dy_wgrad_reduce_desc_bytes": (i32, []),
    "dy_wgrad_reduce_desc_fill": (i32, [vp, vp, i32, vp, i32, i32, i32, i32, i32, i32, i32, i32, i32]),
    "dy_wgrad_reduce_batched": (i32, [vp, i32, i32, vp]),
    "dy_match_predictions": (i32, [vp, vp, vp, vp, vp, i32, vp, vp, i32, i32, i32, i32, vp, vp, vp, vp]),
    "dy_box_iou": (i32, [vp, i32, vp, i32, vp, vp]),
    "dy_conv_num_partials": (i32, [i32, i32, i32, i32, i32, i32, i32, i32]),
    "dy_wgrad_workspace": (i32, [i32, i32, i32, i32, i32, i32, i32, ip, lp]),
    "dy_conv_wgrad": (i32, [vp, i32, vp, i32, vp, vp, i32, i32, i32, i32, i32, i32, i32, i32, vp]),
    "dy_stem_grid": (i32, [i32, i32, i32]),
    "dy_stem_forward": (i32, [vp, vp, vp, i32, vp, i32, i32, i32, f32, vp]),
    "dy_stem_forward_eval": (i32, [vp, vp, vp, vp, i32, i32, i32, i32, f32, i32, vp]),
    "dy_stem_wgrad_bn": (i32, [vp, vp, i32, vp, i32, vp, vp, vp, vp, f32, vp, i32, i32, i32, f32, vp]),
    "dy_conv_wgrad_bias": (i32, [vp, i32, vp, i32, vp, vp, vp, i32, i32, i32, i32, i32, i32, i32, i32, vp]),
    "dy_wgrad_reduce_desc_bias": (i32, [vp, vp, vp, i32]),
    "dy_conv_wgrad_bn": (i32, [vp, i32, vp, i32, vp, i32, vp, vp, vp, vp, vp, f32, vp, vp, i32, i32, i32, i32, i32, i32, i32, i32, vp]),
    "dy_conv_wgrad_ld_bn": (i32, [vp, i32, vp, i32, vp, i32, vp, vp, vp, vp, vp, f32, vp, vp, i32, i32, i32, i32, i32, i32, i32, i32, vp]),
    "dy_ldconv_sample": (i32, [vp, i32, vp, i32, vp, vp, i32, i32, i32, i32, i32, i32, i32, i32, i32, vp]),
    "dy_ldconv_sample_backward": (i32, [vp, i32, vp, i32, vp, vp, i32, vp, vp, i32, i32, i32, i32, i32, i32, i32, i32, i32, vp]),
    "dy_ldconv_sample_backward_gather": (i32, [vp, i32, vp, i32, vp, vp, i32, vp, i32, i32, vp, vp, i32, vp, i32, i32, i32, i32, i32, i32, i32, i32, i32, vp]),
    "dy_f32_to_f16_add": (i32, [vp, vp, i32, i64, i32, i32, vp]),
    "dy_pack_weights_ld": (i32, [vp, vp, i32, i32, i32, i32, i32, vp]),
    "dy_conv_wgrad_ld": (i32, [vp, i32, vp, i32, vp, vp, i32, i32, i32, i32, i32, i32, i32, i32, vp]),
    "dy_bn_finalize": (i32, [vp, i32, f32, vp, i32, f32, vp, i32, f32, vp, vp, vp, vp, vp, i32, f32, f32, f32, i32, vp]),
    "dy_bn_eval_coef": (i32, [vp, vp, vp, vp, vp, i32, f32, vp]),
    "dy_bn_act_apply": (i32, [vp, i32, vp, i32, vp, i32, vp, i64, i32, i32, vp]),
    "dy_bn_act_apply_acc": (i32, [vp, i32, vp, i32, vp, i32, vp, vp, vp, vp, vp, vp, i64, i32, i32, f32, f32, f32, vp]),
    "dy_bn_act_bwd_reduce_acc": (i32, [vp, i32, vp, i32, vp, vp, i64, i32, i32, vp, i32, i32, vp]),
    "dy_bn_act_bwd_apply_acc": (i32, [vp, i32, vp, i32, vp, i32, vp, vp, vp, vp, i64, i32, i32, f32, vp]),
    "dy_bn_act_bwd_reduce": (i32, [vp, i32, vp, i32, vp, vp, i32, i64, i32, i32, ip, vp]),
    "dy_bn_bwd_finalize": (i32, [vp, i32, vp, vp, vp, i32, f32, i32, vp]),
    "dy_bn_act_bwd_apply": (i32, [vp, i32, vp, i32, vp, i32, vp, vp, i64, i32, i32, i32, vp]),
    "dy_bn_finalize_ld": (i32, [vp, i32, i32, vp, vp, vp, vp, vp, i32, f32, f32, f32, i32, vp, vp]),
    "dy_bn_act_apply_c": (i32, [vp, i32, vp, i32, vp, i32, vp, i64, i32, i32, vp]),
    "dy_bn_act_bwd_reduce_c": (i32, [vp, i32, vp, i32, vp, vp, i32, i64, i32, i32, ip, vp]),
    "dy_bn_bwd_finalize_ld": (i32, [vp, i32, i32, vp, vp, vp, i32, f32, i32, vp]),
    "dy_bn_act_bwd_apply_c": (i32, [vp, i32, vp, i32, vp, i32, vp, vp, i64, i32, i32, i32, vp]),
    "dy_pad_f32": (i32, [vp, i32, vp, i32, vp]),
    "dy_import_image": (i32, [vp, vp, i32, i32, i32, i32, i32, f32, vp]),
    "dy_crop_letterbox_u8": (i32, [vp, i32, i32, vp, vp, i32, i32, vp, vp]),
    "dy_refine_select": (i32, [vp, vp, vp, vp, vp, i32, C.c_float, C.c_float, vp, vp, vp]),
    "dy_nms_hard": (i32, [vp, vp, vp, i32, C.c_float, vp, vp]),
    "dy_crop_letterbox_u8_multi": (i32, [vp, vp, vp, vp, vp, vp, i32, i32, vp, vp]),
    "dy_refine_select_multi": (i32, [vp, vp, vp, vp, vp, vp, vp, i32, vp, vp, vp]),
    "dy_two_stage_merge": (i32, [vp, vp, vp, vp, vp, vp, i32, f32, vp, vp, f32, i32, vp, vp, vp, vp]),
    "dy_tile_gather_f32": (i32, [vp, vp, vp, vp, vp, vp, vp, i32, i32, vp, vp]),
    "dy_tile_merge": (i32, [vp, vp, vp, vp, vp, i32, i32, i32, f32, i32, i32, vp, vp, vp, vp, vp]),
    "dy_warp_import_u8": (i32, [vp, vp, vp, i32, i32, i32, vp]),
    "dy_warp_slot_bytes": (i32, []),
    "dy_import_image_u8": (i32, [vp, vp, i32, i32, i32, i32, vp, vp, vp, vp]),
    "dy_add": (i32, [vp, i32, vp, i32, vp, i32, vp, i32, i64, i32, vp]),
    "dy_upsample2x": (i32, [vp, i32, vp, i32, i32, i32, i32, i32, i32, i32, vp]),
    "dy_space_to_depth": (i32, [vp, i32, vp, i32, i32, i32, i32, i32, i32, i32, vp]),
    "dy_dysample_supported": (i32, [i32, i32, i32]),
    "dy_dysample": (i32, [vp, i32, vp, i32, vp, i32, i32, i32, i32, i32, i32, i32, vp]),
    "dy_dysample_backward": (i32, [vp, i32, vp, i32, vp, i32, vp, i32, i32, vp, vp, i32, vp, i32, i32, i32, i32, i32, i32, i32, vp]),
    "dy_carafe_supported": (i32, [i32, i32, i32]),
    "dy_carafe": (i32, [vp, i32, vp, i32, vp, i32, i32, i32, i32, i32, vp]),
    "dy_carafe_backward": (i32, [vp, i32, vp, i32, vp, i32, vp, i32, i32, vp, i32, i32, i32, i32, i32, vp]),
    "dy_maxpool5": (i32, [vp, i32, vp, i32, vp, i32, i32, i32, i32, vp]),
    "dy_maxpool5_backward": (i32, [vp, i32, vp, vp, i32, i32, i32, i32, i32, i32, vp]),
    "dy_bn_group_max": (i32, []),
    "dy_bn_act_apply_acc_split": (i32, [vp, i32, vp, i32, vp, i32, i32, vp, vp, vp, vp, vp, vp, i64, i32, i32, f32, f32, f32, vp]),
    "dy_bn_act_bwd_reduce_acc_split": (i32, [vp, i32, vp, i32, i32, vp, i32, vp, vp, i64, i32, i32, vp]),
    "dy_conv1x1_wgrad_bn_planes": (i32, [C.POINTER(DySegs), vp, i32, vp, vp, i32, i32, vp, i32, vp, vp, vp, vp, vp, f32, vp, vp, i32, i32, i32,
                                         i32, i32, i32, vp]),
    "dy_conv1x1_wgrad_dgrad_supported": (i32, [i32, i32, i32, i32, i32]),
    "dy_wgrad_dgrad_kernel_name": (i32, [i32, i32, i32, i32, i32, i32, C.c_char_p, i32]),
    "dy_conv1x1_wgrad_dgrad_bn": (i32, [vp, i32, vp, i32, vp, i32, vp, vp, vp, vp, f32, vp, vp, vp, vp, i32, i32, i32, i32, i32, i32, i32, i32, vp]),
    "dy_conv1x1_wgrad_dgrad_bn_segs": (i32, [C.POINTER(DySegs), vp, i32, vp, i32, vp, vp, vp, vp, f32, vp, vp, vp, C.POINTER(DySegs), i32, i32,
                                             i32, i32, i32, i32, vp]),
    "dy_conv1x1_wgrad_dgrad_bn_planes": (i32, [C.POINTER(DySegs), vp, i32, vp, vp, i32, i32, vp, i32, vp, vp, vp, vp, f32, vp, vp, vp, vp, i32, i32,
                                               C.POINTER(DySegs), i32, i32, i32, i32, i32, i32, vp]),
    "dy_conv1x1_dgrad_bn_supported": (i32, [i32, i32, i32, i32, i32]),
    "dy_dgrad_only_kernel_name": (i32, [i32, i32, i32, i32, i32, i32, C.c_char_p, i32]),
    "dy_conv1x1_dgrad_bn": (i32, [vp, vp, i32, i32, vp, i32, vp, vp, f32, vp, vp, i32, i32, C.POINTER(DySegs), i32, i32, i32, i32, i32, vp]),
    "dy_bn_act_apply_acc_group": (i32, [i32, vp, vp, vp, vp, vp, vp, vp, vp, vp, vp, vp, vp, vp, vp, vp, vp]),
    "dy_bn_act_bwd_reduce_acc_group": (i32, [i32, vp, vp, vp, vp, vp, vp, vp, vp, vp]),
    "dy_bn_act_bwd_reduce_rows": (i32, [vp, i32, vp, i32, vp, vp, i32, i32, i32, i32, vp, i32, i32, vp]),
    "dy_head_box_decode": (i32, [vp, i32, vp, vp, vp, vp, i32, i32, i32, i32, i32, i32, i32, vp]),
    "dy_cls_head_supported": (i32, [i32, i32]),
    "dy_cls_head_slabs": (i32, []),
    "dy_cls_head_forward": (i32, [vp, i32, vp, vp, vp, vp, i64, i32, i32, vp]),
    "dy_cls_head_backward": (i32, [vp, i32, vp, vp, vp, vp, i32, i32, vp, vp, i64, i32, i32, vp]),
    "dy_head_box_decode_levels": (i32, [i32, vp, vp, vp, vp, vp, vp, i32, vp, i32, vp, vp, i32, i32, vp]),
    "dy_conv1x1_rows_backward_levels": (i32, [i32, vp, vp, vp, vp, vp, vp, i32, vp, vp, vp, vp, vp, vp, vp, i32, vp, vp, i32, i32, vp]),
    "dy_cls_head_forward_levels": (i32, [i32, vp, vp, vp, vp, vp, vp, vp, i32, i32, vp]),
    "dy_cls_head_backward_levels": (i32, [i32, vp, vp, vp, vp, vp, vp, vp, vp, vp, vp, vp, i32, i32, vp]),
    "dy_conv1x1_rows_supported": (i32, [i32, i32]),
    "dy_conv1x1_rows_slabs": (i32, [i32, i32, i32]),
    "dy_conv1x1_rows_backward": (i32, [vp, i32, vp, vp, i32, vp, i32, i32, vp, vp, i32, i32, vp, vp, i32, i32, i32, i32, i32, vp]),
    "dy_sppf_pool3_supported": (i32, [i32, i32, i32]),
    "dy_sppf_pool3": (i32, [vp, i32, i32, vp, vp, vp, i32, i32, i32, vp]),
    "dy_sppf_pool3_backward": (i32, [vp, i32, i32, vp, vp, vp, i32, i32, i32, i32, i32, i32, vp]),
    "dy_scalseq_tail": (i32, [vp, i32, vp, i32, vp, i32, vp, i32, vp, i32, vp, i32, i32, i32, i32, vp]),
    "dy_scalseq_tail_backward": (i32, [vp, i32, vp, i32, vp, i32, vp, i32, vp, i32, vp, vp, vp, i32, i32, i32, i32, i32,
                                       i32, i32, ip, vp]),
    "dy_scalseq_tail_backward_all": (i32, [vp, i32, vp, i32, vp, i32, vp, i32, vp, i32, vp, i32, vp, i32, vp, vp, vp, i32, i32,
                                           i32, i32, i32, i32, ip, vp]),
    "dy_scalseq_bwd_grid_cap": (i32, [i32]),
    "dy_zoom_pool": (i32, [vp, i32, vp, i32, i32, i32, i32, i32, vp]),
    "dy_zoom_pool_backward": (i32, [vp, i32, vp, i32, vp, i32, i32, i32, i32, i32, i32, vp]),
    "dy_copy_slice": (i32, [vp, i32, vp, i32, i64, i32, vp]),
    "dy_fill_zero": (i32, [vp, sz, vp]),
    "dy_loss_workspace_bytes": (sz, [i32, i32, i32]),
    "dy_loss_workspace_layout": (i32, [i32, i32, i32, C.POINTER(sz), C.POINTER(sz), C.POINTER(sz)]),
    "dy_detection_loss": (i32, [C.POINTER(DyLossArgs), vp]),
    "dy_tal_assign": (i32, [vp, ip, ip, C.POINTER(f32), i32, i32, i32, i32, i32, vp, vp, vp, vp, vp, vp, vp, vp]),
    "dy_head_infer_supported": (i32, [i32, i32, i32, i32]),
    "dy_head_infer_levels": (i32, [i32, vp, vp, vp, vp, vp, vp, vp, vp, vp, vp, vp, i32, i32, i32, vp, vp]),
    "dy_head_infer_levels_logits": (i32, [i32, vp, vp, vp, vp, vp, vp, vp, vp, vp, vp, vp, i32, i32, i32, vp, vp, vp, vp]),
    "dy_decode_predictions": (i32, [vp, vp, ip, ip, C.POINTER(f32), i32, i32, i32, i32, vp, vp]),
    "dy_nms_candidates": (i32, [vp, i32, i32, i32, f32, i32, vp, i32, vp, vp, vp, vp, i32, vp]),
    "dy_nms_presort_workspace": (sz, [i32, i32]),
    "dy_nms_presort": (i32, [vp, vp, vp, vp, i32, i32, i32, vp, vp, vp, vp, vp]),
    "dy_soft_nms": (i32, [vp, vp, vp, vp, vp, vp, vp, vp, i32, i32, f32, f32, f32, f32, vp]),
    "dy_set_hyper": (i32, [vp, vp, vp]),
    "dy_optimizer_step": (i32, [vp, vp, vp, vp, vp, i64, i64, i64, vp, vp, vp, i64, vp, vp, vp, i32, vp]),
    "dy_optimizer_step_seg": (i32, [vp, vp, vp, vp, vp, i64, lp, vp, vp, vp, i64, vp, vp, vp, i32, vp]),
    "dy_axpy_f32": (i32, [vp, vp, f32, i64, vp]),
    "dy_scale_img": (i32, [vp, i32, i32, i32, i32, i32, i32, i32, i32, vp, vp]),
    "dy_tta_merge": (i32, [i32, C.POINTER(vp), ip, ip, ip, C.POINTER(f32), ip, i32, i32, i32, i32, vp, vp]),
    "dy_bootstrap_ap": (i32, [vp, vp, vp, vp, vp, i32, i32, i32, i32, vp, vp, vp]),
    "dy_confusion_matrix": (i32, [vp, vp, i32, vp, vp, vp, i32, vp, i32, i32, i32, i32, f32, f32, i32, vp, vp, vp]),
    "dy_count_fp": (i32, [vp, vp, vp, vp, vp, i32, f32, C.c_double, vp, vp, vp]),
}

_LIB = None


def lib():
    global _LIB
    if _LIB is None:
        if not os.path.exists(LIB_PATH):
            raise RuntimeError(
                f"{LIB_PATH} not found. The DEAL-YOLO hot path has no CPU/PyTorch fallback: build the HIP library "
                f"first (python -c 'import __graft_entry__ as g; g.build()' or `make -C experiment-yolo_amd/csrc`).")
        L = C.CDLL(LIB_PATH)
        for name, (res, args) in SIGNATURES.items():
            fn = getattr(L, name)
            fn.restype, fn.argtypes = res, args
        if L.dy_segs_bytes() != C.sizeof(DySegs):
            raise RuntimeError(f"{LIB_PATH} lays DySegs out in {L.dy_segs_bytes()} bytes, this binding in {C.sizeof(DySegs)}: rebuild the library")
        if L.dy_loss_args_bytes() != C.sizeof(DyLossArgs):
            raise RuntimeError(f"{LIB_PATH} was built with a DyLossArgs of {L.dy_loss_args_bytes()} bytes, this binding lays out "
                               f"{C.sizeof(DyLossArgs)}: rebuild the library (make -C experiment-yolo_amd/csrc)")
        _LIB = L
    return _LIB


def check(rc, name):
    if rc != 0:
        raise RuntimeError(f"{name} failed: {_ERR.get(rc, rc)}")
```

include/dealyolo_hip.h:

```cpp
#ifndef DEALYOLO_HIP_H
#define DEALYOLO_HIP_H

#include <stddef.h>
#include <stdint.h>

#ifdef __cplusplus
extern "C" {
#endif

#ifndef __HIP__
typedef struct ihipStream_t* hipStream_t;
#endif

#define DY_OK 0
#define DY_ERR_ARG (-1)
#define DY_ERR_LAUNCH (-2)
#define DY_ERR_ALIGN (-3)
#define DY_ERR_CAPACITY (-4)

#define DY_MAX_SEGS 8
typedef struct DySegs {
  int nseg;
  int c_end[DY_MAX_SEGS];
  int ld[DY_MAX_SEGS];
  int acc[DY_MAX_SEGS];
  const void* ptr[DY_MAX_SEGS];
} DySegs;
int dy_segs_bytes(void);

#define DY_EPI_STATS 1
#define DY_EPI_BIAS 2
#define DY_EPI_SILU 4
#define DY_EPI_F32OUT 8
#define DY_EPI_ACCUM 16
#define DY_EPI_STATS_ACC 32
#define DY_BN_COPIES 16

#define DY_ACT_NONE 0
#define DY_ACT_SILU 1
#define DY_ACT_LEAKY 2

int dy_abi_version(void);

int dy_conv_geometry(int cin, int cout, int ks, int stride, int* cin_p, int* cout_p, int* cc, int* nch, int* mt,
                     int* ngroups, int* ksteps, int* packed_elems);
int dy_pack_weights(const float* w, const float* scale, void* out, int cout, int cin, int ks, int stride,
                    int transposed, hipStream_t stream);
int dy_pack_desc_bytes(void);
int dy_pack_desc_fill(void* desc, const float* w, const float* scale, void* out, int cout, int cin, int ks, int stride,
                      int transposed, int ld_taps, int ld_cphys, int first_block);
int dy_pack_weights_batched(const void* descs_device, int n, int total_blocks, hipStream_t stream);
int dy_conv_forward(const void* x, int ldx, const void* w_packed, const float* bias, void* y, int ldy, float* partials,
                    int n, int h, int w, int cin, int cout, int ks, int stride, int dil, int out_h, int out_w, int epi,
                    int* num_partials, hipStream_t stream);
int dy_conv_num_partials(int n, int h, int w, int cin, int cout, int ks, int stride, int dil);
int dy_conv_res_supported(int cin, int cout, int ks, int stride);
int dy_conv_forward_res(const void* x, int ldx, const void* w_packed, const float* bias, const void* res, int ldres, void* y, int ldy,
                        int n, int h, int w, int cin, int cout, int ks, int stride, hipStream_t stream);
int dy_conv_red_supported(int cin, int cout, int ks);
int dy_conv_input_grad_red(const void* dy, int lddy, const void* w_packed_t, void* dx, int lddx, int n, int h, int w, int cin, int cout,
                           int ks, const void* raw, int ldraw, const float* coef, double* acc, int C, hipStream_t stream);
int dy_conv_kernel_name(int cin, int cout, int ks, int stride, char* out, int cap);
int dy_conv_kernel_name_at(int cin, int cout, int ks, int stride, int out_w, int dil, int epi, char* out, int cap);

int dy_wgrad_workspace(int n, int h, int w, int cin, int cout, int ks, int stride, int* nslabs, long* slab_elems);
int dy_wgrad_kernel_name(int cin, int cout, int ks, int stride, char* out, int cap);
int dy_wgrad_kernel_name_at(int n, int h, int w, int cin, int cout, int ks, int stride, char* out, int cap);
int dy_conv_wgrad(const void* x, int ldx, const void* dy, int lddy, float* slabs, float* dw, int n, int h, int w,
                  int cin, int cout, int ks, int stride, int accumulate, hipStream_t stream);
int dy_conv_wgrad_bn(const void* x, int ldx, const void* dy, int lddy, const void* raw, int ldraw, void* draw, const float* coef,
                     const double* acc, float* dgamma, float* dbeta, float count, float* slabs, float* dw, int n, int h, int w,
                     int cin, int cout, int ks, int stride, int accumulate, hipStream_t stream);
int dy_conv_wgrad_ld_bn(const void* x, int ldx, const void* dy, int lddy, const void* raw, int ldraw, void* draw,
                        const float* coef, const double* acc, float* dgamma, float* dbeta, float count, float* slabs, float* dw,
                        int n, int h, int w, int cout, int ld_cin, int ld_taps, int ld_cphys, int accumulate, hipStream_t stream);
int dy_conv1x1_segs_supported(int cin, int cout, const DySegs* xs);
int dy_conv1x1_segs_kernel_name(int cin, int cout, const DySegs* xs, char* out, int cap);
int dy_conv1x1_kernel_name_live(int cin, int cout, int n, int h, int w, int epi, const DySegs* xs, const DySegs* ys, char* out, int cap);
int dy_conv1x1_forward_segs(const DySegs* xs, const void* w_packed, const float* bias, void* y, int ldy, float* partials, int n, int h,
                            int w, int cin, int cout, int epi, hipStream_t stream);
int dy_conv1x1_input_grad_segs(const void* dy, int lddy, const void* w_packed_t, const DySegs* dxs, int n, int h, int w, int cin, int cout,
                               hipStream_t stream);
int dy_conv1x1_wgrad_bn_segs(const DySegs* xs, const void* dy, int lddy, const void* raw, int ldraw, void* draw, const float* coef,
                             const double* acc, float* dgamma, float* dbeta, float count, float* slabs, float* dw, int n, int h, int w,
                             int cin, int cout, int accumulate, hipStream_t stream);
int dy_bn_act_apply_acc_split(const void* x, int ldx, void* y, int ldy, void* y2, int ldy2, int csplit, const double* acc,
                              const float* gamma, const float* beta, float* running_mean, float* running_var, float* coef, long npix,
                              int C, int act, float count, float eps, float momentum, hipStream_t stream);
int dy_bn_act_bwd_reduce_acc_split(const void* dy, int lddy, const void* dy2, int lddy2, int csplit, const void* x, int ldx,
                                   const float* coef, double* acc, long npix, int C, int act, hipStream_t stream);
int dy_conv1x1_wgrad_bn_planes(const DySegs* xs, const void* x, int ldx, const void* dy, const void* dy2, int lddy, int csplit,
                               const void* raw, int ldraw, void* draw, const float* coef, const double* acc, float* dgamma,
                               float* dbeta, float count, float* slabs, float* dw, int n, int h, int w, int cin, int cout,
                               int accumulate, hipStream_t stream);
int dy_conv1x1_wgrad_dgrad_supported(int n, int h, int w, int cin, int cout);
int dy_wgrad_dgrad_kernel_name(int n, int h, int w, int cin, int cout, int segs, char* out, int cap);
int dy_conv1x1_wgrad_dgrad_bn(const void* x, int ldx, const void* dy, int lddy, const void* raw, int ldraw, const float* coef,
                              const double* acc, float* dgamma, float* dbeta, float count, float* slabs, float* dw,
                              const void* w_packed_t, void* dx, int lddx, int dx_accumulate, int n, int h, int w, int cin, int cout,
                              int accumulate, hipStream_t stream);
int dy_conv1x1_wgrad_dgrad_bn_segs(const DySegs* xs, const void* dy, int lddy, const void* raw, int ldraw, const float* coef,
                                   const double* acc, float* dgamma, float* dbeta, float count, float* slabs, float* dw,
                                   const void* w_packed_t, const DySegs* dxs, int n, int h, int w, int cin, int cout, int accumulate,
                                   hipStream_t stream);
int dy_conv1x1_wgrad_dgrad_bn_planes(const DySegs* xs, const void* x, int ldx, const void* dy, const void* dy2, int lddy, int csplit,
                                     const void* raw, int ldraw, const float* coef, const double* acc, float* dgamma, float* dbeta,
                                     float count, float* slabs, float* dw, const void* w_packed_t, void* dx, int lddx,
                                     int dx_accumulate, const DySegs* dxs, int n, int h, int w, int cin, int cout, int accumulate,
                                     hipStream_t stream);
int dy_conv1x1_dgrad_bn_supported(int n, int h, int w, int cin, int cout);
int dy_dgrad_only_kernel_name(int n, int h, int w, int cin, int cout, int segs, char* out, int cap);
int dy_conv1x1_dgrad_bn(const void* dy, const void* dy2, int lddy, int csplit, const void* raw, int ldraw, const float* coef,
                        const double* acc, float count, const void* w_packed_t, void* dx, int lddx, int dx_accumulate,
                        const DySegs* dxs, int n, int h, int w, int cin, int cout, hipStream_t stream);
int dy_stem_grid(int n, int h, int w);
int dy_stem_forward(const float* img_nchw, const float* weight, void* raw, int ldraw, double* acc, int n, int h, int w, float mul,
                    hipStream_t stream);
int dy_stem_forward_eval(const float* img_nchw, const float* weight, const float* bias, void* y, int ldy, int n, int h, int w, float mul,
                         int silu, hipStream_t stream);
int dy_stem_wgrad_bn(const float* img_nchw, const void* dy, int lddy, const void* raw, int ldraw, const float* coef,
                     const double* acc, float* dgamma, float* dbeta, float count, float* slabs, int n, int h, int w, float mul,
                     hipStream_t stream);
int dy_conv_wgrad_bias(const void* x, int ldx, const void* dy, int lddy, double* bias_acc, float* slabs, float* dw, int n, int h, int w,
                       int cin, int cout, int ks, int stride, int accumulate, hipStream_t stream);
int dy_wgrad_reduce_desc_bias(void* desc, const double* bias_acc, float* dbias, int c);
int dy_wgrad_reduce_desc_bytes(void);
int dy_wgrad_reduce_desc_fill(void* desc, const float* slabs, int nslabs, float* dw, int cin, int cout, int ks, int stride,
                              int accumulate, int ld_taps, int ld_cphys, int ld_cin, int first_block);
int dy_wgrad_reduce_batched(const void* descs_device, int n, int total_blocks, hipStream_t stream);

int dy_ldconv_sample(const void* x, int ldx, const float* off, int ldoff, const int* pn, void* xo, int ldxo, int n, int H,
                     int W, int h, int w, int C, int Np, int stride, hipStream_t stream);
int dy_ldconv_sample_backward(const void* x, int ldx, const float* off, int ldoff, const int* pn, const void* dxo,
                              int lddxo, float* dx32, void* doff, int lddoff, int n, int H, int W, int h, int w, int C,
                              int Np, int stride, hipStream_t stream);
int dy_ldconv_sample_backward_gather(const void* x, int ldx, const float* off, int ldoff, const int* pn, const void* dxo,
                                     int lddxo, void* dx, int lddx, int accumulate, float* dx32, void* doff, int lddoff,
                                     void* scratch, int rmax, int n, int H, int W, int h, int w, int C, int Np, int stride,
                                     hipStream_t stream);
int dy_f32_to_f16_add(const float* src, void* dst, int ld, long npix, int C, int accumulate, hipStream_t stream);
int dy_pack_weights_ld(const float* w, void* out, int cout, int cin, int ld_taps, int ld_cphys, int transposed,
                       hipStream_t stream);
int dy_conv_wgrad_ld(const void* x, int ldx, const void* dy, int lddy, float* slabs, float* dw, int n, int h, int w,
                     int cout, int ld_cin, int ld_taps, int ld_cphys, int accumulate, hipStream_t stream);

int dy_bn_finalize(const float* p0, int n0, float w0, const float* p1, int n1, float w1, const float* p2, int n2,
                   float w2, const float* gamma, const float* beta, float* running_mean, float* running_var,
                   float* coef, int C, float count, float eps, float momentum, int update_running, hipStream_t stream);
int dy_bn_eval_coef(const float* gamma, const float* beta, const float* running_mean, const float* running_var,
                    float* coef, int C, float eps, hipStream_t stream);
int dy_bn_act_apply(const void* x, int ldx, const void* res, int ldr, void* y, int ldy, const float* coef, long npix,
                    int C, int act, hipStream_t stream);
int dy_bn_act_apply_acc(const void* x, int ldx, const void* res, int ldr, void* y, int ldy, const double* acc,
                        const float* gamma, const float* beta, float* running_mean, float* running_var, float* coef,
                        long npix, int C, int act, float count, float eps, float momentum, hipStream_t stream);
int dy_bn_act_bwd_reduce_acc(const void* dy, int lddy, const void* x, int ldx, const float* coef, double* acc, long npix,
                             int C, int act, void* res_grad, int ldrg, int res_accumulate, hipStream_t stream);
int dy_bn_group_max(void);
int dy_bn_act_apply_acc_group(int n, const void* const* x, const int* ldx, void* const* y, const int* ldy, const double* const* acc,
                              const float* const* gamma, const float* const* beta, float* const* running_mean, float* const* running_var,
                              float* const* coef, const long* npix, const int* C, const float* count, const float* eps,
                              const float* momentum, hipStream_t stream);
int dy_bn_act_bwd_reduce_acc_group(int n, const void* const* dy, const int* lddy, const void* const* x, const int* ldx,
                                   const float* const* coef, double* const* acc, const long* npix, const int* C, hipStream_t stream);
int dy_bn_act_bwd_reduce_rows(const void* dy, int lddy, const void* x, int ldx, const float* coef, double* acc, int n, int hw, int C,
                              int act, const int* assigned, int A, int a0, hipStream_t stream);
int dy_bn_act_bwd_apply_acc(const void* dy, int lddy, const void* x, int ldx, void* dx, int lddx, const float* coef,
                            const double* acc, float* dgamma, float* dbeta, long npix, int C, int act, float count,
                            hipStream_t stream);
int dy_bn_act_bwd_reduce(const void* dy, int lddy, const void* x, int ldx, const float* coef, float* partials,
                         int max_partials, long npix, int C, int act, int* nparts, hipStream_t stream);
int dy_bn_bwd_finalize(const float* partials, int nparts, float* dgamma, float* dbeta, float* bwdcoef, int C,
                       float count, int accumulate, hipStream_t stream);
int dy_bn_act_bwd_apply(const void* dy, int lddy, const void* x, int ldx, void* dx, int lddx, const float* coef,
                        const float* bwdcoef, long npix, int C, int act, int frozen_stats, hipStream_t stream);

int dy_bn_finalize_ld(const float* part, int nparts, int ldp, const float* gamma, const float* beta, float* running_mean,
                      float* running_var, float* coef, int C, float count, float eps, float momentum, int update_running,
                      long long* num_batches_tracked, hipStream_t stream);
int dy_bn_act_apply_c(const void* x, int ldx, const void* res, int ldr, void* y, int ldy, const float* coef, long npix, int C,
                      int act, hipStream_t stream);
int dy_bn_act_bwd_reduce_c(const void* dy, int lddy, const void* x, int ldx, const float* coef, float* partials, int max_partials,
                           long npix, int C, int act, int* nparts, hipStream_t stream);
int dy_bn_bwd_finalize_ld(const float* partials, int nparts, int ldp, float* dgamma, float* dbeta, float* bwdcoef, int C,
                          float count, int accumulate, hipStream_t stream);
int dy_bn_act_bwd_apply_c(const void* dy, int lddy, const void* x, int ldx, void* dx, int lddx, const float* coef,
                          const float* bwdcoef, long npix, int C, int act, int frozen_stats, hipStream_t stream);
int dy_pad_f32(const float* src, int n, float* dst, int n_pad, hipStream_t stream);

int dy_import_image(const float* x_nchw, void* y, int n, int c, int h, int w, int cp, float mul, hipStream_t stream);
int dy_import_image_u8(const void* x, void* y, int n, int h, int w, int cp, const void* flip, const int* index,
                       const float* hsv, hipStream_t stream);
int dy_warp_import_u8(const void* pool, const void* slots, void* y, int n, int s, int cp, hipStream_t stream);
int dy_warp_slot_bytes(void);
int dy_add(const void* a, int lda, const void* b, int ldb, const void* c, int ldc, void* y, int ldy, long npix, int C,
           hipStream_t stream);
int dy_upsample2x(const void* x, int ldx, void* y, int ldy, int n, int h, int w, int C, int backward, int accumulate,
                  hipStream_t stream);
int dy_space_to_depth(void* x, int ldx, void* y, int ldy, int n, int h, int w, int C, int backward, int accumulate,
                      hipStream_t stream);
int dy_dysample_supported(int C, int G, int s);
int dy_dysample(const void* x, int ldx, const float* off, int ldoff, void* y, int ldy, int n, int H, int W, int C, int G, int s,
                hipStream_t stream);
int dy_dysample_backward(const void* x, int ldx, const float* off, int ldoff, const void* dy, int lddy, void* dx, int lddx,
                         int accumulate, float* dx32, void* doff, int lddoff, void* scratch, int rmax, int n, int H, int W, int C,
                         int G, int s, hipStream_t stream);
int dy_carafe_supported(int C, int k_up, int scale);
int dy_carafe(const void* x, int ldx, const void* logits, int ldl, void* y, int ldy, int n, int H, int W, int C, hipStream_t stream);
int dy_carafe_backward(const void* x, int ldx, const void* logits, int ldl, const void* dy, int lddy, void* dx, int lddx,
                       int accumulate, void* dlogits, int lddl, int n, int H, int W, int C, hipStream_t stream);
int dy_maxpool5(const void* x, int ldx, void* y, int ldy, void* argmax, int n, int h, int w, int C, hipStream_t stream);
int dy_maxpool5_backward(const void* dy, int lddy, const void* argmax, void* dx, int lddx, int n, int h, int w, int C,
                         int accumulate, hipStream_t stream);
int dy_sppf_pool3_supported(int h, int w, int C);
int dy_sppf_pool3(void* cat, int ld, int C, void* arg0, void* arg1, void* arg2, int n, int h, int w, hipStream_t stream);
int dy_sppf_pool3_backward(void* gcat, int ld, int C, const void* arg0, const void* arg1, const void* arg2, int n, int h, int w,
                           int acc0, int acc1, int acc2, hipStream_t stream);
int dy_scalseq_tail(const void* r0, int ld0, const void* r1, int ld1, const void* r2, int ld2, const void* res,
                    int ldres, void* y, int ldy, const float* coef, int n, int h, int w, int C, hipStream_t stream);
int dy_scalseq_tail_backward(const void* r0, int ld0, const void* r1, int ld1, const void* r2, int ld2, const void* dy,
                             int lddy, void* dr, int lddr, const float* coef, const float* bwdcoef, float* partials,
                             int max_partials, int n, int h, int w, int C, int level, int mode, int* nparts,
                             hipStream_t stream);
int dy_scalseq_tail_backward_all(const void* r0, int ld0, const void* r1, int ld1, const void* r2, int ld2,
                                 const void* dy, int lddy, void* dr0, int lddr0, void* dr1, int lddr1, void* dr2,
                                 int lddr2, const float* coef, const float* bwdcoef, float* partials, int max_partials,
                                 int n, int h, int w, int C, int mode, int* nparts, hipStream_t stream);
int dy_scalseq_bwd_grid_cap(int cap);
int dy_zoom_pool(const void* x, int ldx, void* y, int ldy, int n, int h, int w, int C, hipStream_t stream);
int dy_zoom_pool_backward(const void* x, int ldx, const void* dy, int lddy, void* dx, int lddx, int n, int h, int w, int C,
                          int accumulate, hipStream_t stream);
int dy_copy_slice(const void* x, int ldx, void* y, int ldy, long npix, int C, hipStream_t stream);
int dy_fill_zero(void* p, size_t bytes, hipStream_t stream);

typedef struct DyLossArgs {
  int nl, B, nc, ncp, nmax;
  const float* box[4];
  const float* cls[4];
  void* dbox[4];
  void* dcls[4];
  int H[4], W[4];
  float stride[4];
  const float* t_batch_idx;
  const float* t_cls;
  const float* t_boxes;
  int n_targets;
  const int* n_targets_dev;
  float img_w, img_h;
  float hyp_box, hyp_cls, hyp_dfl;
  int use_wiou, use_nwd;
  float iou_ratio;
  const float* gscale;
  float* scalars;
  void* workspace;
  int dbox_rows_only;
  int box_from_input;
  const void* box_in[4];
  int box_in_ld[4];
  const float* box_w[4];
  const float* box_b[4];
  const float* box_in_coef[4];
  int box_family;
  int box_ltype;
  int box_fm;
  int box_modifier;
  float inner_ratio;
  float focaler_d, focaler_u;
  float shape_scale;
  float piou_lambda;
} DyLossArgs;
#define DY_BOX_FAMILY_LEGACY 0
#define DY_BOX_FAMILY_WISE 1
#define DY_BOX_FAMILY_BBOX 2
#define DY_BOX_IOU 0
#define DY_BOX_WIOU 1
#define DY_BOX_EIOU 2
#define DY_BOX_GIOU 3
#define DY_BOX_DIOU 4
#define DY_BOX_CIOU 5
#define DY_BOX_SIOU 6
#define DY_BOX_SHAPEIOU 7
#define DY_BOX_PIOU 8
#define DY_BOX_PIOU2 9
#define DY_BOX_MPDIOU 10
#define DY_BOX_FM_V1 1
#define DY_BOX_FM_V2 2
#define DY_BOX_FM_V3 3
#define DY_BOX_MOD_PLAIN 0
#define DY_BOX_MOD_INNER 1
#define DY_BOX_MOD_FOCALER 2
int dy_loss_args_bytes(void);
size_t dy_loss_workspace_bytes(int B, int A, int nmax);
int dy_loss_workspace_layout(int B, int A, int nmax, size_t* off_pred_box, size_t* off_asg_gt, size_t* off_tscore);
int dy_detection_loss(const DyLossArgs* args, hipStream_t stream);
int dy_head_box_decode(const void* x, int ldx, const float* x_coef, const float* weight, const float* bias, float* pred_box, int A, int a0,
                       int n, int h, int w, int cin, int cout, hipStream_t stream);
int dy_cls_head_supported(int cin, int nc);
int dy_cls_head_slabs(void);
int dy_cls_head_forward(const void* x, int ldx, const float* x_coef, const float* weight, const float* bias, float* logits, long npix,
                        int cin, int nc, hipStream_t stream);
int dy_cls_head_backward(const void* x, int ldx, const float* x_coef, const void* dy, const float* weight, void* dx, int lddx,
                         int dx_accumulate, float* slabs, double* bias_acc, long npix, int cin, int nc, hipStream_t stream);
int dy_head_box_decode_levels(int nl, const void* const* x, const int* ldx, const float* const* x_coef, const float* const* weight,
                              const float* const* bias, float* pred_box, int A, const int* a0, int n, const int* h, const int* w, int cin,
                              int cout, hipStream_t stream);
int dy_conv1x1_rows_backward_levels(int nl, const void* const* x, const int* ldx, const float* const* x_coef, const void* const* dy,
                                    const int* lddy, const int* assigned, int A, const int* a0, const float* const* weight, void* const* dx,
                                    const int* lddx, const int* dx_accumulate, float* const* slabs, double* const* bias_acc, int n,
                                    const int* h, const int* w, int cin, int cout, hipStream_t stream);
int dy_cls_head_forward_levels(int nl, const void* const* x, const int* ldx, const float* const* x_coef, const float* const* weight,
                               const float* const* bias, float* const* logits, const long* npix, int cin, int nc, hipStream_t stream);
int dy_cls_head_backward_levels(int nl, const void* const* x, const int* ldx, const float* const* x_coef, const void* const* dy,
                                const float* const* weight, void* const* dx, const int* lddx, const int* dx_accumulate, float* const* slabs,
                                double* const* bias_acc, const long* npix, int cin, int nc, hipStream_t stream);
int dy_conv1x1_rows_supported(int cin, int cout);
int dy_conv1x1_rows_slabs(int n, int h, int w);
int dy_conv1x1_rows_backward(const void* x, int ldx, const float* x_coef, const void* dy, int lddy, const int* assigned, int A, int a0,
                             const float* weight, void* dx, int lddx, int dx_accumulate, float* slabs, double* bias_acc, int n,
                             int h, int w, int cin, int cout, hipStream_t stream);
int dy_tal_assign(const float* const* scores, const int* H, const int* W, const float* stride, int nl, int B, int nc, int ncp,
                  int n, const float* pd_boxes_grid, const int* gt_labels, const float* gt_bboxes, const int* mask_gt, int* asg_gt,
                  float* tscore, void* workspace, hipStream_t stream);

int dy_head_infer_supported(int cin_box, int cout_box, int cin_cls, int nc);
int dy_head_infer_levels(int nl, const void* const* x_box, const int* ld_box, const float* const* w_box, const float* const* b_box,
                         const void* const* x_cls, const int* ld_cls, const float* const* w_cls, const float* const* b_cls, const int* h,
                         const int* w, const float* stride, int n, int cin_cls, int nc, float* y, hipStream_t stream);
int dy_head_infer_levels_logits(int nl, const void* const* x_box, const int* ld_box, const float* const* w_box, const float* const* b_box,
                                const void* const* x_cls, const int* ld_cls, const float* const* w_cls, const float* const* b_cls,
                                const int* h, const int* w, const float* stride, int n, int cin_cls, int nc, float* y,
                                float* const* box_logits, float* const* cls_logits, hipStream_t stream);
int dy_decode_predictions(const float* const* box, const float* const* cls, const int* H, const int* W,
                          const float* stride, int nl, int B, int nc, int ncp, float* y, hipStream_t stream);
int dy_nms_candidates(const float* pred, int B, int nc, int A, float conf, int multi_label, const int* classes,
                      int n_classes, float* cbox, float* cscore, float* ccls, int* ccount, int cap, hipStream_t stream);
size_t dy_nms_presort_workspace(int B, int max_nms);
int dy_nms_presort(const float* cbox, const float* cscore, const float* ccls, int* count, int B, int cap, int max_nms, float* obox,
                   float* oscore, float* ocls, void* workspace, hipStream_t stream);
int dy_soft_nms(const float* boxes, float* scores, const float* cls, const int* count, int* order_a, int* order_b,
                int* keep, int* nkeep, int B, int cap, float iou_thr, float sigma, float score_thr, float class_offset,
                hipStream_t stream);

int dy_optimizer_step(float* params, const float* grads, float* mom, float* adam_v, float* ema, long n, long g0_end,
                      long g1_end, const unsigned char* frozen, const float* buffers, float* ema_buffers,
                      long n_buffers, const float* hyper, float* state, float* partials, int mode, hipStream_t stream);
int dy_optimizer_step_seg(float* params, const float* grads, float* mom, float* adam_v, float* ema, long n, const long* seg_ends,
                          const unsigned char* frozen, const float* buffers, float* ema_buffers, long n_buffers, const float* hyper,
                          float* state, float* partials, int mode, hipStream_t stream);
int dy_set_hyper(float* hyper_dev, const float* host_values16, hipStream_t stream);
int dy_axpy_f32(float* y, const float* x, float a, long n, hipStream_t stream);

int dy_match_predictions(const float* preds, const int* pred_off, const float* t_batch_idx, const float* t_cls,
                         const float* t_boxes, int n_targets, const float* geom, const float* iouv, int niou, int B,
                         int img_h, int img_w, unsigned char* tp, float* predn, int* status, hipStream_t stream);
int dy_box_iou(const float* box1, int n, const float* box2, int m, float* out, hipStream_t stream);

int dy_crop_letterbox_u8(const void* img, int H, int W, const int* rects, const int* geom, int K, int S, void* out,
                         hipStream_t stream);
int dy_refine_select(const float* dets, const int* offsets, const float* orig, const int* rects, const float* scale, int K,
                     float img_w, float img_h, float* out, int* found, hipStream_t stream);
int dy_nms_hard(const float* boxes, const float* scores, const float* labels, int n, float iou_thr, void* keep,
                hipStream_t stream);

int dy_crop_letterbox_u8_multi(const void* pool, const long* img_off, const int* img_hw, const int* crop_img, const int* rects,
                               const int* geom, int K, int S, void* out, hipStream_t stream);
int dy_refine_select_multi(const float* dets, const int* offsets, const float* orig, const int* rects, const float* scale,
                           const int* crop_img, const int* img_hw, int K, float* out, int* found, hipStream_t stream);
int dy_two_stage_merge(float* rows, const int* row_off, const float* refined, const int* found, const int* crop_row,
                       const int* crop_off, int aligned, float nms_iou, const float* labels, const int* lab_off, float match_iou,
                       int N, void* keep, int* counts, int* status, hipStream_t stream);

int dy_scale_img(const float* x, int B, int H, int W, int flip, int Ho, int Wo, int Hp, int Wp, float* out, hipStream_t stream);
int dy_tta_merge(int n_pass, const float* const* y_ptrs, const int* A, const int* col_lo, const int* col_hi, const float* scale,
                 const int* flip, int B, int no, int H, int W, float* out, hipStream_t stream);

int dy_bootstrap_ap(const unsigned short* tp_bits, const int* det_img, const int* cls_off, const int* lab_cnt,
                    const unsigned short* mult, int D, int n_img, int nc, int S, double* ap, int* nl, hipStream_t stream);

int dy_confusion_matrix(const float* predn, const int* pred_off, int n_preds, const float* t_batch_idx, const float* t_cls,
                        const float* t_boxes, int n_targets, const float* geom, int B, int img_h, int img_w, int nc, float conf_thr,
                        float iou_thres, int skip_unlabelled, int* matrix, int* status, hipStream_t stream);
int dy_count_fp(const float* dets, const int* det_off, const double* labels, const int* lab_off, const int* wh, int B, float conf_thr,
                double iou_thr, int* fp, int* status, hipStream_t stream);

int dy_tile_gather_f32(const void* pool, const long* img_off, const int* img_hw, const int* tile_img, const int* rects, const int* geom,
                       const float* lut, int K, int S, float* out, hipStream_t stream);
#define DY_TILE_MERGE_MAX_ROWS 8192
int dy_tile_merge(const float* rows, const int* row_off, const int* row_tile, const float* tiles, const int* img_hw, int N, int Kt,
                  int max_rows, float thr, int metric, int agnostic, float* out, int* order, int* nkeep, int* status,
                  hipStream_t stream);

#ifdef __cplusplus
}
#endif
#endif
```

Before: 6059 images/s.

## Use 8-wave blocks for wide 3x3 wgrad and software-pipeline stem image loads

Two unrelated changes. First, the wide 3x3 weight-gradient kernel becomes templated on wave count, and its large-channel forms now launch with 512 threads by default. Accumulator columns are split across more waves, which cuts per-thread register pressure and may raise occupancy. Second, the stem forward and weight-gradient kernels prefetch the next tile's image rows into registers as float4 while computing the current tile, and the wgrad path uses a new LDS layout, which adds register and LDS cost.

```diff
diff --git a/experiment-yolo_amd/csrc/conv_wgrad.hip b/experiment-yolo_amd/csrc/conv_wgrad.hip
--- a/experiment-yolo_amd/csrc/conv_wgrad.hip
+++ b/experiment-yolo_amd/csrc/conv_wgrad.hip
@@ -50,18 +50,30 @@
   return (nci * mtc <= 1) ? 8 : ((nci + mtc <= 4) ? 4 : 2);
 }
 
-template <int KS, int STRIDE, int NCI, int MTC, int BNF>
-__global__ __launch_bounds__(256, (BNF & 8) ? 3 : ((KS == 3 && NCI * MTC >= 16) ? 1 : 2)) void conv_wgrad_kernel(const WgArgs a) {
+static constexpr __host__ __device__ bool wg_wide_block(int ks, int nci, int mtc) { return ks == 3 && nci * mtc >= 16; }
+#define DY_WGRAD_WIDE_DEFAULT 1
+#define DY_WGRAD_ALT 16
+static constexpr __host__ __device__ int wg_nw(int ks, int nci, int mtc, int bnfx) {
+  return (wg_wide_block(ks, nci, mtc) && (bnfx & ~DY_WGRAD_ALT) <= 2 && (((bnfx & DY_WGRAD_ALT) != 0) != (DY_WGRAD_WIDE_DEFAULT != 0))) ? 8 : 4;
+}
+template <int KS, int STRIDE, int NCI, int MTC, int BNFX>
+__global__ __launch_bounds__(64 * wg_nw(KS, NCI, MTC, BNFX),
+                             (BNFX & 8) ? 3 : (wg_nw(KS, NCI, MTC, BNFX) == 8 ? 2 : (wg_wide_block(KS, NCI, MTC) ? 1 : 2)))
+void conv_wgrad_kernel(const WgArgs a) {
+  constexpr int BNF = BNFX & ~DY_WGRAD_ALT;
+  constexpr int NW = wg_nw(KS, NCI, MTC, BNFX);
+  static_assert(!(BNFX & DY_WGRAD_ALT) || (wg_wide_block(KS, NCI, MTC) && BNF <= 2), "two wave counts: the wide 3x3 blocks only");
+  constexpr int NT = 64 * NW;
   constexpr bool FLAT = (KS == 1);
   constexpr bool DG = (BNF & 4) != 0;
   constexpr bool NOX = (BNF & 8) != 0;
   static_assert(!NOX || DG, "the form without X exists for the fused input gradient only");
   constexpr bool BN1 = ((BNF & 3) == 1 || (BNF & 3) == 3);
   constexpr bool XSEG = ((BNF & 3) == 3);
-  static_assert(!DG || (KS == 1 && BN1), "the fused input gradient exists for the 1x1 BatchNorm forms");
+  static_assert(!DG || (KS == 1 && BN1 && NW == 4), "the fused input gradient exists for the 1x1 BatchNorm forms");
   constexpr int TAPS = KS * KS;
   constexpr int NCOL = NCI * TAPS;
-  constexpr int CPW = (NCOL + 3) / 4;
+  constexpr int CPW = (NCOL + NW - 1) / NW;
   constexpr int TH = wg_th(KS, STRIDE, NCI, MTC), TW = 32;
   constexpr int HWX = FLAT ? TH * TW : (TW - 1) * STRIDE + KS;
   constexpr int HHX = FLAT ? 1 : (TH - 1) * STRIDE + KS;
@@ -73,7 +85,7 @@
   __shared__ __attribute__((aligned(16))) char smem[XBYTES + YBYTES];
   char* const sx = smem;
   char* const sy = smem + XBYTES;
-  __shared__ __attribute__((aligned(16))) float sbn[BN1 ? 4 * COUT_C : (BNF == 2 ? 256 * 8 : 4)];
+  __shared__ __attribute__((aligned(16))) float sbn[BN1 ? 4 * COUT_C : (BNF == 2 ? NT * 8 : 4)];
   float bsum[8] = {0.f, 0.f, 0.f, 0.f, 0.f, 0.f, 0.f, 0.f};
   (void)bsum;
   constexpr int DKS = MTC == 4 ? 2 : (MTC == 3 ? 3 : 1), DCPK = (MTC & 1) ? 16 : 32;
@@ -100,7 +112,7 @@
   (void)acc;
 
   constexpr int NGX = HHX * HWX * (CIN_C / 8), NGY = TH * TW * (COUT_C / 8);
-  constexpr int NPX = NOX ? 1 : (NGX + 255) / 256, NPY = (NGY + 255) / 256;
+  constexpr int NPX = NOX ? 1 : (NGX + NT - 1) / NT, NPY = (NGY + NT - 1) / NT;
   uint4 pfx[NPX], pfy[NPY];
   uint4 pfr[BN1 ? NPY : 1];
   unsigned roff[BN1 ? NPY : 1];
@@ -114,7 +126,7 @@
   (void)pfx; (void)xoff;
 #pragma unroll
   for (int i = 0; i < NPX; ++i) {
-    const int id = tid + i * 256;
+    const int id = tid + i * NT;
     const int pixel = id / CPGX, part = id - pixel * CPGX;
     const bool ok = !NOX && id < NGX && ci0 + part * 8 < a.cin_r8;
     const int hy = FLAT ? 0 : pixel / HWX, hx = FLAT ? pixel : pixel - hy * HWX;
@@ -131,7 +143,7 @@
   if (XIN) {
 #pragma unroll
     for (int i = 0; i < NPX; ++i) {
-      const int id = tid + i * 256;
+      const int id = tid + i * NT;
       const int part = id % CPGX, ch = ci0 + part * 8;
       int sg = 0;
       while (sg + 1 < a.xs.nseg && ch >= a.xs.c_end[sg]) ++sg;
@@ -144,7 +156,7 @@
   }
 #pragma unroll
   for (int i = 0; i < NPY; ++i) {
-    const int id = tid + i * 256;
+    const int id = tid + i * NT;
     const int pixel = id / CPGY, part = id - pixel * CPGY;
     const bool ok = id < NGY && co0 + part * 8 < a.cout_r8;
     const int ty = FLAT ? 0 : pixel / TW, tx = FLAT ? pixel : pixel - ty * TW;
@@ -156,7 +168,7 @@
     if (BN1) roff[i] = ok ? (unsigned)(((ty * a.Wo + tx) * a.ldraw + co0 + part * 8) * 2) : NEVER;
   }
   if (BN1) {
-    for (int c = tid; c < COUT_C; c += 256) {
+    for (int c = tid; c < COUT_C; c += NT) {
       const int ch = co0 + c;
       float sc = 0.f, sh = 0.f, kb = 0.f, kc = 0.f;
       if (ch < a.cout) {
@@ -255,7 +267,7 @@
         const float invW = 1.0f / (float)a.W, invH = 1.0f / (float)a.H;
 #pragma unroll
         for (int i = 0; i < NPX; ++i) {
-          const int lp = (tid + i * 256) / CPGX;
+          const int lp = (tid + i * NT) / CPGX;
           long gp = p0 + lp;
           const bool inside = gp < a.npix;
           if ((xup >> i) & 1u) {
@@ -299,7 +311,7 @@
       } else {
 #pragma unroll
         for (int i = 0; i < NPX; ++i) {
-          const int hx = ((tid + i * 256) / CPGX) % HWX;
+          const int hx = ((tid + i * NT) / CPGX) % HWX;
           pfx[i] = ld16(rx, (unsigned)(ix0 + hx) < (unsigned)a.W ? xoff[i] + ox : NEVER);
         }
       }
@@ -309,7 +321,7 @@
       } else {
 #pragma unroll
         for (int i = 0; i < NPY; ++i) {
-          const int tx = ((tid + i * 256) / CPGY) % TW;
+          const int tx = ((tid + i * NT) / CPGY) % TW;
           pfy[i] = ld16(ry, ox0 + tx < a.Wo ? yoff[i] + oy : NEVER);
         }
       }
@@ -323,7 +335,7 @@
         for (int i = 0; i < NPY; ++i) {
           unsigned off = roff[i] == NEVER ? NEVER : roff[i] + ornext;
           if (!xfull) {
-            const int tx = ((tid + i * 256) / CPGY) % TW;
+            const int tx = ((tid + i * NT) / CPGY) % TW;
             off = ox0 + tx < a.Wo ? off : NEVER;
           }
           pfr[i] = ld16(rr, off);
@@ -341,7 +353,7 @@
     __syncthreads();
 #pragma unroll
     for (int i = 0; i < NPX; ++i) {
-      const int id = tid + i * 256;
+      const int id = tid + i * NT;
       if (!NOX && id < NGX) *reinterpret_cast<uint4*>(sx + (id / (CIN_C / 8)) * PSX + (id % (CIN_C / 8)) * 16) = pfx[i];
     }
     if (BN1) {
@@ -350,7 +362,7 @@
       const auto rd = __builtin_amdgcn_make_buffer_rsrc(FLAT ? a.draw : a.draw + (size_t)ncur * a.Ho * a.Wo * a.ldraw, 0, (int)nbytes, 0x00020000);
 #pragma unroll
       for (int i = 0; i < NPY; ++i) {
-        const int id = tid + i * 256;
+        const int id = tid + i * NT;
         const int part = id % CPGY;
         const bool valid = (vcur >> i) & 1u;
         const float* cf = sbn + part * 8;
@@ -364,7 +376,7 @@
     } else {
 #pragma unroll
       for (int i = 0; i < NPY; ++i) {
-        const int id = tid + i * 256;
+        const int id = tid + i * NT;
         if (id < NGY) *reinterpret_cast<uint4*>(sy + (id / (COUT_C / 8)) * PSY + (id % (COUT_C / 8)) * 16) = pfy[i];
         if (BNF == 2 && id < NGY) {
           const half8 v = *reinterpret_cast<const half8*>(&pfy[i]);
@@ -400,7 +412,7 @@
       }
     };
     auto load_b = [&](int buf, int r, int c) {
-      const int col = wave + 4 * c;
+      const int col = wave + NW * c;
       if (col < NCOL) {
         const int cit = col / TAPS, tap = col - cit * TAPS;
         const int dy = tap / KS, dx = tap - dy * KS;
@@ -427,7 +439,7 @@
         if (c + 1 < CPW) load_b((lin + 1) & 1, r, c + 1);
         else if (r + 1 < TH) load_b((lin + 1) & 1, r + 1, 0);
         __builtin_amdgcn_sched_barrier(0);
-        if (wave + 4 * c < NCOL) {
+        if (wave + NW * c < NCOL) {
 #pragma unroll
           for (int m = 0; m < MTC; ++m)
             acc[NOX ? 0 : m][NOX ? 0 : c] = __builtin_amdgcn_mfma_f32_16x16x32_f16(af[r & 1][m], bf[lin & 1], acc[NOX ? 0 : m][NOX ? 0 : c], 0, 0, 0);
@@ -504,7 +516,7 @@
     if (tid < COUT_C && co0 + tid < a.cout) {
       const int part = tid >> 3, j = tid & 7;
       float t = 0.f;
-      for (int k = part; k < 256; k += CPGY) t += sbn[k * 8 + j];
+      for (int k = part; k < NT; k += CPGY) t += sbn[k * 8 + j];
       unsafeAtomicAdd(const_cast<double*>(a.acc) + (size_t)(blockIdx.x % DY_BN_COPIES) * a.cout + co0 + tid, (double)t);
     }
   }
@@ -512,7 +524,7 @@
   float* slab = a.slabs + (size_t)blockIdx.x * TAPS * a.cout_p * a.cin_p;
 #pragma unroll
   for (int c = 0; c < CPW; ++c) {
-    const int col = wave + 4 * c;
+    const int col = wave + NW * c;
     if (col < NCOL) {
       const int cit = col / TAPS, tap = col - cit * TAPS;
 #pragma unroll
@@ -622,6 +634,20 @@
   return DY_OK;
 }
 
+static bool wgrad_wide() {
+  const char* e = getenv("DY_WGRAD_WIDE");
+  return (e && (e[0] == '0' || e[0] == '1') && !e[1]) ? e[0] == '1' : DY_WGRAD_WIDE_DEFAULT != 0;
+}
+template <int KS, int STRIDE, int NCI, int MTC, int BNF>
+static void launch_wgrad_form(const WgArgs& a, int gx, int gy, hipStream_t s) {
+  if constexpr (wg_wide_block(KS, NCI, MTC) && BNF <= 2) {
+    if (wgrad_wide() != (DY_WGRAD_WIDE_DEFAULT != 0)) {
+      hipLaunchKernelGGL((conv_wgrad_kernel<KS, STRIDE, NCI, MTC, BNF + DY_WGRAD_ALT>), dim3(gx, gy), dim3(64 * wg_nw(KS, NCI, MTC, BNF + DY_WGRAD_ALT)), 0, s, a);
+      return;
+    }
+  }
+  hipLaunchKernelGGL((conv_wgrad_kernel<KS, STRIDE, NCI, MTC, BNF>), dim3(gx, gy), dim3(64 * wg_nw(KS, NCI, MTC, BNF)), 0, s, a);
+}
 template <int KS, int STRIDE, int NCI, int MTC>
 static int launch_wgrad(const WgArgs& a, int gx, int gy, hipStream_t s) {
   if (a.wt) {
@@ -636,10 +662,10 @@
   } else if (a.raw && a.xs.nseg > 0) {
     if constexpr (KS == 1) hipLaunchKernelGGL((conv_wgrad_kernel<KS, STRIDE, NCI, MTC, 3>), dim3(gx, gy), dim3(256), 0, s, a);
     else return DY_ERR_ARG;
-  } else if (a.raw) hipLaunchKernelGGL((conv_wgrad_kernel<KS, STRIDE, NCI, MTC, 1>), dim3(gx, gy), dim3(256), 0, s, a);
-  else if (a.acc && MTC != 3) hipLaunchKernelGGL((conv_wgrad_kernel<KS, STRIDE, NCI, MTC, 2>), dim3(gx, gy), dim3(256), 0, s, a);
+  } else if (a.raw) launch_wgrad_form<KS, STRIDE, NCI, MTC, 1>(a, gx, gy, s);
+  else if (a.acc && MTC != 3) launch_wgrad_form<KS, STRIDE, NCI, MTC, 2>(a, gx, gy, s);
   else if (a.acc) return DY_ERR_ARG;
-  else hipLaunchKernelGGL((conv_wgrad_kernel<KS, STRIDE, NCI, MTC, 0>), dim3(gx, gy), dim3(256), 0, s, a);
+  else launch_wgrad_form<KS, STRIDE, NCI, MTC, 0>(a, gx, gy, s);
   DY_CHECK_LAUNCH();
   return DY_OK;
 }
@@ -722,11 +748,14 @@
                            int cin, int cout, int ks, int stride, int accumulate, int ld_taps, int ld_cphys, int ld_cin,
                            hipStream_t stream, const WgBnHost* bn = nullptr);
 
+static int wgrad_kernel_bnf0(int ks, int nci, int mtc) {
+  return (wg_wide_block(ks, nci, mtc) && wgrad_wide() != (DY_WGRAD_WIDE_DEFAULT != 0)) ? DY_WGRAD_ALT : 0;
+}
 extern "C" int dy_wgrad_kernel_name(int cin, int cout, int ks, int stride, char* out, int cap) {
   if (!out || cap < 8) return DY_ERR_ARG;
   int cp, op, nci, mtc;
   wgrad_geometry(cin, cout, ks, stride, &cp, &op, &nci, &mtc);
-  snprintf(out, cap, "conv_wgrad_kernel<%d, %d, %d, %d, 0>", ks, stride, nci, mtc);
+  snprintf(out, cap, "conv_wgrad_kernel<%d, %d, %d, %d, %d>", ks, stride, nci, mtc, wgrad_kernel_bnf0(ks, nci, mtc));
   return DY_OK;
 }
 
@@ -735,7 +764,7 @@
   int cp, op, nci, mtc;
   wgrad_geometry(cin, cout, ks, stride, &cp, &op, &nci, &mtc,
                  (long)n * ((h + 2 * (ks / 2) - ks) / stride + 1) * ((w + 2 * (ks / 2) - ks) / stride + 1));
-  snprintf(out, cap, "conv_wgrad_kernel<%d, %d, %d, %d, 0>", ks, stride, nci, mtc);
+  snprintf(out, cap, "conv_wgrad_kernel<%d, %d, %d, %d, %d>", ks, stride, nci, mtc, wgrad_kernel_bnf0(ks, nci, mtc));
   return DY_OK;
 }
 
diff --git a/experiment-yolo_amd/csrc/stem.hip b/experiment-yolo_amd/csrc/stem.hip
--- a/experiment-yolo_amd/csrc/stem.hip
+++ b/experiment-yolo_amd/csrc/stem.hip
@@ -55,8 +55,74 @@
 typedef _Float16 half4_ __attribute__((ext_vector_type(4)));
 typedef uint2 __attribute__((aligned(4))) uint2_a4;
 
+#define STEM_NF4 17
+#define STEM_FWD_PIPE_WAVES 6
+#define STEM_RPT (256 / STEM_NF4)
+#define STEM_PF ((3 * STEM_IH + STEM_RPT - 1) / STEM_RPT)
+static __device__ __forceinline__ void stem_fetch4(const StemArgs& a, float4 (&v)[STEM_PF], int n, int oy0, int bx) {
+  const int iy0 = 2 * oy0 - 1, ixa = 2 * STEM_TW * bx - 4;
+  const float* img = a.img + (size_t)n * 3 * a.H * a.W;
+  const int r0 = threadIdx.x / STEM_NF4, f = threadIdx.x - r0 * STEM_NF4, ix = ixa + 4 * f;
+  const bool xok = r0 < STEM_RPT && (unsigned)ix < (unsigned)a.W;
+#pragma unroll
+  for (int u = 0; u < STEM_PF; ++u) {
+    const int r = r0 + u * STEM_RPT, c = (r >= STEM_IH) + (r >= 2 * STEM_IH), iy = iy0 + r - c * STEM_IH;
+    const bool ok = xok && r < 3 * STEM_IH && (unsigned)iy < (unsigned)a.H;
+    v[u] = ok ? *reinterpret_cast<const float4*>(img + ((size_t)c * a.H + iy) * a.W + ix) : make_float4(0.f, 0.f, 0.f, 0.f);
+  }
+}
+typedef _Float16 half2_ __attribute__((ext_vector_type(2)));
+static __device__ __forceinline__ void stem_put4(float mul, f16 (*s_in)[STEM_IH][STEM_IP], const float4 (&v)[STEM_PF]) {
+  const int r0 = threadIdx.x / STEM_NF4, f = threadIdx.x - r0 * STEM_NF4;
+#pragma unroll
+  for (int u = 0; u < STEM_PF; ++u) {
+    const int r = r0 + u * STEM_RPT;
+    if (r0 < STEM_RPT && r < 3 * STEM_IH) {
+      f16* dst = &s_in[0][0][0] + r * STEM_IP + 4 * f;
+      if (f) {
+        dst[-3] = (f16)(v[u].x * mul);
+        *reinterpret_cast<half2_*>(dst - 2) = (half2_){(f16)(v[u].y * mul), (f16)(v[u].z * mul)};
+      }
+      dst[0] = (f16)(v[u].w * mul);
+    }
+  }
+}
+
 template <bool INFER>
-__global__ __launch_bounds__(256) void stem_fwd_kernel(StemArgs a) {
+static __device__ __forceinline__ void stem_fwd_tile(const StemArgs& a, const f16* s_flat, const half4_ (&af)[3], const int (&goff)[3], const f32x4& b4,
+                                                     int n, int oy0, int ox0, f32x4& s1, f32x4& s2) {
+  const int wave = threadIdx.x >> 6, lane = threadIdx.x & 63, p = lane & 15, q = lane >> 4;
+#pragma unroll
+  for (int nt = 0; nt < 4; ++nt) {
+    const int ty = wave * 2 + (nt >> 1), px = (nt & 1) * 16 + p;
+    f32x4 acc = {0.f, 0.f, 0.f, 0.f};
+#pragma unroll
+    for (int ks = 0; ks < 3; ++ks) {
+      union { uint2 u; half4_ h; } bf;
+      const uint2_a4* src = reinterpret_cast<const uint2_a4*>(s_flat + goff[ks] + (2 * ty) * STEM_IP + 2 * px);
+      bf.u.x = src->x;
+      bf.u.y = src->y;
+      acc = __builtin_amdgcn_mfma_f32_16x16x16f16(af[ks], bf.h, acc, 0, 0, 0);
+    }
+    const int oy = oy0 + ty, ox = ox0 + px;
+    if (oy < a.Ho && ox < a.Wo) {
+      union { half4_ h; uint2 u; } o;
+      if (INFER) {
+        acc += b4;
+        if (a.silu) acc = (f32x4){silu_f(acc[0]), silu_f(acc[1]), silu_f(acc[2]), silu_f(acc[3])};
+      }
+      o.h = __builtin_convertvector(acc, half4_);
+      *reinterpret_cast<uint2*>(a.raw + (((size_t)n * a.Ho + oy) * a.Wo + ox) * a.ldraw + q * 4) = o.u;
+      if (!INFER) {
+        s1 += acc;
+        s2 += acc * acc;
+      }
+    }
+  }
+}
+
+template <bool INFER, bool PIPE>
+static __device__ __forceinline__ void stem_fwd_body(const StemArgs& a) {
   __shared__ __attribute__((aligned(16))) f16 s_in[3][STEM_IH][STEM_IP];
   __shared__ float s_red[4][2][STEM_CO];
   const int tid = threadIdx.x, wave = tid >> 6, lane = tid & 63, p = lane & 15, q = lane >> 4;
@@ -75,40 +141,24 @@
   const f16* s_flat = &s_in[0][0][0];
   for (int e = tid; e < 3 * STEM_IH * (STEM_IP - STEM_IW); e += 256)
     (&s_in[0][0][0])[(e / (STEM_IP - STEM_IW)) * STEM_IP + STEM_IW + e % (STEM_IP - STEM_IW)] = (f16)0.f;
+  float4 pf[STEM_PF];
+  if constexpr (PIPE) {
+    const int bx = blockIdx.x % a.tiles_x, t2 = blockIdx.x / a.tiles_x;
+    stem_fetch4(a, pf, t2 / a.tiles_y, (t2 % a.tiles_y) * STEM_TH, bx);
+  }
   for (int tile = blockIdx.x; tile < a.ntiles; tile += gridDim.x) {
     const int bx = tile % a.tiles_x, t2 = tile / a.tiles_x;
     const int by = t2 % a.tiles_y, n = t2 / a.tiles_y;
     const int oy0 = by * STEM_TH, ox0 = bx * STEM_TW;
     __syncthreads();
-    stem_stage(a, s_in, n, oy0, ox0);
+    if constexpr (PIPE) stem_put4(a.mul, s_in, pf);
+    else stem_stage(a, s_in, n, oy0, ox0);
     __syncthreads();
-#pragma unroll
-    for (int nt = 0; nt < 4; ++nt) {
-      const int ty = wave * 2 + (nt >> 1), px = (nt & 1) * 16 + p;
-      f32x4 acc = {0.f, 0.f, 0.f, 0.f};
-#pragma unroll
-      for (int ks = 0; ks < 3; ++ks) {
-        union { uint2 u; half4_ h; } bf;
-        const uint2_a4* src = reinterpret_cast<const uint2_a4*>(s_flat + goff[ks] + (2 * ty) * STEM_IP + 2 * px);
-        bf.u.x = src->x;
-        bf.u.y = src->y;
-        acc = __builtin_amdgcn_mfma_f32_16x16x16f16(af[ks], bf.h, acc, 0, 0, 0);
-      }
-      const int oy = oy0 + ty, ox = ox0 + px;
-      if (oy < a.Ho && ox < a.Wo) {
-        union { half4_ h; uint2 u; } o;
-        if (INFER) {
-          acc += b4;
-          if (a.silu) acc = (f32x4){silu_f(acc[0]), silu_f(acc[1]), silu_f(acc[2]), silu_f(acc[3])};
-        }
-        o.h = __builtin_convertvector(acc, half4_);
-        *reinterpret_cast<uint2*>(a.raw + (((size_t)n * a.Ho + oy) * a.Wo + ox) * a.ldraw + q * 4) = o.u;
-        if (!INFER) {
-          s1 += acc;
-          s2 += acc * acc;
-        }
-      }
-    }
+    if constexpr (PIPE) if (tile + (int)gridDim.x < a.ntiles) {
+      const int nx = tile + gridDim.x, nbx = nx % a.tiles_x, nt2 = nx / a.tiles_x;
+      stem_fetch4(a, pf, nt2 / a.tiles_y, (nt2 % a.tiles_y) * STEM_TH, nbx);
+    }
+    stem_fwd_tile<INFER>(a, s_flat, af, goff, b4, n, oy0, ox0, s1, s2);
   }
   if (INFER) return;
 #pragma unroll
@@ -127,9 +177,43 @@
   }
 }
 
+template <bool INFER>
+__global__ __launch_bounds__(256) void stem_fwd_kernel(StemArgs a) { stem_fwd_body<INFER, false>(a); }
+template <bool INFER>
+__global__ __launch_bounds__(256, STEM_FWD_PIPE_WAVES) void stem_fwd_pipe_kernel(StemArgs a) { stem_fwd_body<INFER, true>(a); }
+
 #define STEM_DP (STEM_TH * STEM_TW + 8)
-__global__ __launch_bounds__(256) void stem_wgrad_bn_kernel(StemArgs a) {
-  __shared__ __attribute__((aligned(16))) f16 s_in[3][STEM_IH][STEM_IP];
+#define STEM_KP 40
+static __device__ __forceinline__ void stem_put4_k(float mul, f16* s_k, const float4 (&v)[STEM_PF]) {
+  const int r0 = threadIdx.x / STEM_NF4, f = threadIdx.x - r0 * STEM_NF4;
+#pragma unroll
+  for (int u = 0; u < STEM_PF; ++u) {
+    const int r = r0 + u * STEM_RPT;
+    if (r0 < STEM_RPT && r < 3 * STEM_IH) {
+      f16* k0 = s_k + r * 3 * STEM_KP + 2 * f;
+      const f16 h1 = (f16)(v[u].y * mul), h3 = (f16)(v[u].w * mul);
+      if (f) {
+        *reinterpret_cast<half2_*>(k0 + STEM_KP - 2) = (half2_){(f16)(v[u].x * mul), (f16)(v[u].z * mul)};
+        *reinterpret_cast<half2_*>(k0 + 2 * STEM_KP - 2) = (half2_){h1, h3};
+        k0[-1] = h1;
+      }
+      k0[0] = h3;
+    }
+  }
+}
+struct StemPix { half8 d0, d1, r0, r1; bool pv; };
+static __device__ __forceinline__ void stem_fetch_pix(const StemArgs& a, StemPix& g, int n, int oy0, int ox0) {
+  const int oy = oy0 + (threadIdx.x >> 5), ox = ox0 + (threadIdx.x & 31);
+  g.pv = oy < a.Ho && ox < a.Wo;
+  const size_t pix = g.pv ? ((size_t)n * a.Ho + oy) * a.Wo + ox : 0;
+  g.d0 = *reinterpret_cast<const half8*>(a.dy + pix * a.lddy);
+  g.d1 = *reinterpret_cast<const half8*>(a.dy + pix * a.lddy + 8);
+  g.r0 = *reinterpret_cast<const half8*>(a.raw + pix * a.ldraw);
+  g.r1 = *reinterpret_cast<const half8*>(a.raw + pix * a.ldraw + 8);
+}
+template <bool PIPE>
+static __device__ __forceinline__ void stem_wgrad_bn_body(const StemArgs& a) {
+  __shared__ __attribute__((aligned(16))) f16 s_in[3][STEM_IH][PIPE ? 3 * STEM_KP : STEM_IP];
   __shared__ __attribute__((aligned(16))) f16 s_d[STEM_CO][STEM_DP];
   __shared__ float s_bn[4][STEM_CO];
   __shared__ float s_acc[4][2][16][16];
@@ -154,38 +238,51 @@
     }
   }
   f32x4 acc[2] = {(f32x4){0.f, 0.f, 0.f, 0.f}, (f32x4){0.f, 0.f, 0.f, 0.f}};
-  for (int e = tid; e < 3 * STEM_IH * (STEM_IP - STEM_IW); e += 256)
-    (&s_in[0][0][0])[(e / (STEM_IP - STEM_IW)) * STEM_IP + STEM_IW + e % (STEM_IP - STEM_IW)] = (f16)0.f;
+  if constexpr (!PIPE)
+    for (int e = tid; e < 3 * STEM_IH * (STEM_IP - STEM_IW); e += 256)
+      (&s_in[0][0][0])[(e / (STEM_IP - STEM_IW)) * STEM_IP + STEM_IW + e % (STEM_IP - STEM_IW)] = (f16)0.f;
   int boff[2];
   bool bok[2];
 #pragma unroll
   for (int nt = 0; nt < 2; ++nt) {
     const int kk = nt * 16 + p, c = kk / 9, r = kk - c * 9, ky = r / 3, kx = r - ky * 3;
     bok[nt] = kk < 27;
-    boff[nt] = bok[nt] ? (c * STEM_IH + ky) * STEM_IP + kx : 0;
-  }
-  const f16* s_in_flat = &s_in[0][0][0];
+    boff[nt] = !bok[nt] ? 0 : (PIPE ? ((c * STEM_IH + ky) * 3 + kx) * STEM_KP : (c * STEM_IH + ky) * STEM_IP + kx);
+  }
+  f16* s_in_flat = &s_in[0][0][0];
+  float4 pf[STEM_PF];
+  StemPix g;
+  if constexpr (PIPE) {
+    const int bx = blockIdx.x % a.tiles_x, t2 = blockIdx.x / a.tiles_x, by = t2 % a.tiles_y, n = t2 / a.tiles_y;
+    stem_fetch_pix(a, g, n, by * STEM_TH, bx * STEM_TW);
+    stem_fetch4(a, pf, n, by * STEM_TH, bx);
+  }
   for (int tile = blockIdx.x; tile < a.ntiles; tile += gridDim.x) {
-    const int bx = tile % a.tiles_x, t2 = tile / a.tiles_x;
-    const int by = t2 % a.tiles_y, n = t2 / a.tiles_y;
-    const int oy0 = by * STEM_TH, ox0 = bx * STEM_TW;
     __syncthreads();
-    const int ty = tid >> 5, tx = tid & 31, oy = oy0 + ty, ox = ox0 + tx;
-    const bool pv = oy < a.Ho && ox < a.Wo;
-    const size_t pix = pv ? ((size_t)n * a.Ho + oy) * a.Wo + ox : 0;
-    const half8 d0 = *reinterpret_cast<const half8*>(a.dy + pix * a.lddy), d1 = *reinterpret_cast<const half8*>(a.dy + pix * a.lddy + 8);
-    const half8 r0 = *reinterpret_cast<const half8*>(a.raw + pix * a.ldraw), r1 = *reinterpret_cast<const half8*>(a.raw + pix * a.ldraw + 8);
-    stem_stage(a, s_in, n, oy0, ox0);
+    if constexpr (PIPE) {
+      stem_put4_k(a.mul, s_in_flat, pf);
+    } else {
+      const int bx = tile % a.tiles_x, t2 = tile / a.tiles_x;
+      const int by = t2 % a.tiles_y, n = t2 / a.tiles_y;
+      const int oy0 = by * STEM_TH, ox0 = bx * STEM_TW;
+      stem_fetch_pix(a, g, n, oy0, ox0);
+      stem_stage(a, s_in, n, oy0, ox0);
+    }
     {
-      half8 o0 = bn_bwd_apply8<DY_ACT_SILU>(d0, r0, s_bn[0], s_bn[1], s_bn[2], s_bn[3]);
-      half8 o1 = bn_bwd_apply8<DY_ACT_SILU>(d1, r1, s_bn[0] + 8, s_bn[1] + 8, s_bn[2] + 8, s_bn[3] + 8);
+      half8 o0 = bn_bwd_apply8<DY_ACT_SILU>(g.d0, g.r0, s_bn[0], s_bn[1], s_bn[2], s_bn[3]);
+      half8 o1 = bn_bwd_apply8<DY_ACT_SILU>(g.d1, g.r1, s_bn[0] + 8, s_bn[1] + 8, s_bn[2] + 8, s_bn[3] + 8);
 #pragma unroll
       for (int j = 0; j < 8; ++j) {
-        s_d[j][tid] = pv ? o0[j] : (f16)0.f;
-        s_d[8 + j][tid] = pv ? o1[j] : (f16)0.f;
+        s_d[j][tid] = g.pv ? o0[j] : (f16)0.f;
+        s_d[8 + j][tid] = g.pv ? o1[j] : (f16)0.f;
       }
     }
     __syncthreads();
+    if constexpr (PIPE) if (tile + (int)gridDim.x < a.ntiles) {
+      const int nx = tile + gridDim.x, bx = nx % a.tiles_x, t2 = nx / a.tiles_x, by = t2 % a.tiles_y, n = t2 / a.tiles_y;
+      stem_fetch_pix(a, g, n, by * STEM_TH, bx * STEM_TW);
+      stem_fetch4(a, pf, n, by * STEM_TH, bx);
+    }
 #pragma unroll
     for (int ks = 0; ks < 2; ++ks) {
       const int row = wave * 2 + ks, pix0 = row * STEM_TW + q * 8;
@@ -193,9 +290,15 @@
       half8 bf[2];
 #pragma unroll
       for (int nt = 0; nt < 2; ++nt) {
-        const f16* b = s_in_flat + boff[nt] + (2 * row) * STEM_IP + 2 * (q * 8);
-#pragma unroll
-        for (int j = 0; j < 8; ++j) bf[nt][j] = bok[nt] ? b[2 * j] : (f16)0.f;
+        if constexpr (PIPE) {
+          const half8 k8 = *reinterpret_cast<const half8*>(s_in_flat + boff[nt] + (2 * row) * 3 * STEM_KP + q * 8);
+#pragma unroll
+          for (int j = 0; j < 8; ++j) bf[nt][j] = bok[nt] ? k8[j] : (f16)0.f;
+        } else {
+          const f16* b = s_in_flat + boff[nt] + (2 * row) * STEM_IP + 2 * (q * 8);
+#pragma unroll
+          for (int j = 0; j < 8; ++j) bf[nt][j] = bok[nt] ? b[2 * j] : (f16)0.f;
+        }
       }
       acc[0] = __builtin_amdgcn_mfma_f32_16x16x32_f16(af, bf[0], acc[0], 0, 0, 0);
       acc[1] = __builtin_amdgcn_mfma_f32_16x16x32_f16(af, bf[1], acc[1], 0, 0, 0);
@@ -213,6 +316,9 @@
     slab[((size_t)tap * 16 + co) * 16 + c] = s;
   }
 }
+
+__global__ __launch_bounds__(256) void stem_wgrad_bn_kernel(StemArgs a) { stem_wgrad_bn_body<false>(a); }
+__global__ __launch_bounds__(256) void stem_wgrad_bn_pipe_kernel(StemArgs a) { stem_wgrad_bn_body<true>(a); }
 
 static int stem_args(StemArgs& a, int n, int h, int w) {
   if (n < 1 || h < 2 || w < 2) return DY_ERR_ARG;
@@ -231,13 +337,25 @@
   return a.ntiles < 1024 ? a.ntiles : 1024;
 }
 
+static bool stem_pipe(const StemArgs& a) {
+  const char* e = getenv("DY_STEM_V1");
+  return !(e && e[0] == '1' && !e[1]) && (a.W & 3) == 0 && ((uintptr_t)a.img & 15) == 0;
+}
+
+extern "C" int dy_stem_pipelined(const float* img_nchw, int w) {
+  StemArgs a{};
+  a.img = img_nchw; a.W = w;
+  return stem_pipe(a) ? 1 : 0;
+}
+
 extern "C" int dy_stem_forward(const float* img_nchw, const float* weight, void* raw, int ldraw, double* acc, int n, int h, int w,
                                float mul, hipStream_t stream) {
   StemArgs a{};
   if (!img_nchw || !weight || !raw || !acc || (ldraw & 7) || ((uintptr_t)raw & 15)) return DY_ERR_ARG;
   if (stem_args(a, n, h, w) != DY_OK) return DY_ERR_ARG;
   a.img = img_nchw; a.w = weight; a.raw = (f16*)raw; a.acc = acc; a.ldraw = ldraw; a.mul = mul;
-  hipLaunchKernelGGL(stem_fwd_kernel<false>, dim3(stem_fwd_grid(a.ntiles)), dim3(256), 0, stream, a);
+  if (stem_pipe(a)) hipLaunchKernelGGL(stem_fwd_pipe_kernel<false>, dim3(stem_fwd_grid(a.ntiles)), dim3(256), 0, stream, a);
+  else hipLaunchKernelGGL(stem_fwd_kernel<false>, dim3(stem_fwd_grid(a.ntiles)), dim3(256), 0, stream, a);
   DY_CHECK_LAUNCH();
   return DY_OK;
 }
@@ -248,7 +366,8 @@
   if (!img_nchw || !weight || !y || (ldy & 7) || ((uintptr_t)y & 15) || (bias && ((uintptr_t)bias & 15))) return DY_ERR_ARG;
   if (stem_args(a, n, h, w) != DY_OK) return DY_ERR_ARG;
   a.img = img_nchw; a.w = weight; a.raw = (f16*)y; a.ldraw = ldy; a.mul = mul; a.bias = bias; a.silu = silu;
-  hipLaunchKernelGGL(stem_fwd_kernel<true>, dim3(stem_fwd_grid(a.ntiles)), dim3(256), 0, stream, a);
+  if (stem_pipe(a)) hipLaunchKernelGGL(stem_fwd_pipe_kernel<true>, dim3(stem_fwd_grid(a.ntiles)), dim3(256), 0, stream, a);
+  else hipLaunchKernelGGL(stem_fwd_kernel<true>, dim3(stem_fwd_grid(a.ntiles)), dim3(256), 0, stream, a);
   DY_CHECK_LAUNCH();
   return DY_OK;
 }
@@ -262,7 +381,8 @@
   if (stem_args(a, n, h, w) != DY_OK) return DY_ERR_ARG;
   a.img = img_nchw; a.dy = (const f16*)dy; a.raw = (f16*)const_cast<void*>(raw); a.coef = coef; a.acc = const_cast<double*>(acc);
   a.dgamma = dgamma; a.dbeta = dbeta; a.slabs = slabs; a.ldraw = ldraw; a.lddy = lddy; a.mul = mul; a.count = count;
-  hipLaunchKernelGGL(stem_wgrad_bn_kernel, dim3(dy_stem_grid(n, h, w)), dim3(256), 0, stream, a);
+  if (stem_pipe(a)) hipLaunchKernelGGL(stem_wgrad_bn_pipe_kernel, dim3(dy_stem_grid(n, h, w)), dim3(256), 0, stream, a);
+  else hipLaunchKernelGGL(stem_wgrad_bn_kernel, dim3(dy_stem_grid(n, h, w)), dim3(256), 0, stream, a);
   DY_CHECK_LAUNCH();
   return DY_OK;
 }
diff --git a/experiment-yolo_amd/ultralytics/hip/__init__.py b/experiment-yolo_amd/ultralytics/hip/__init__.py
--- a/experiment-yolo_amd/ultralytics/hip/__init__.py
+++ b/experiment-yolo_amd/ultralytics/hip/__init__.py
@@ -83,6 +83,7 @@
     "dy_wgrad_workspace": (i32, [i32, i32, i32, i32, i32, i32, i32, ip, lp]),
     "dy_conv_wgrad": (i32, [vp, i32, vp, i32, vp, vp, i32, i32, i32, i32, i32, i32, i32, i32, vp]),
     "dy_stem_grid": (i32, [i32, i32, i32]),
+    "dy_stem_pipelined": (i32, [vp, i32]),
     "dy_stem_forward": (i32, [vp, vp, vp, i32, vp, i32, i32, i32, f32, vp]),
     "dy_stem_forward_eval": (i32, [vp, vp, vp, vp, i32, i32, i32, i32, f32, i32, vp]),
     "dy_stem_wgrad_bn": (i32, [vp, vp, i32, vp, i32, vp, vp, vp, vp, f32, vp, i32, i32, i32, f32, vp]),
diff --git a/include/dealyolo_hip.h b/include/dealyolo_hip.h
--- a/include/dealyolo_hip.h
+++ b/include/dealyolo_hip.h
@@ -114,6 +114,7 @@
                         const double* acc, float count, const void* w_packed_t, void* dx, int lddx, int dx_accumulate,
                         const DySegs* dxs, int n, int h, int w, int cin, int cout, hipStream_t stream);
 int dy_stem_grid(int n, int h, int w);
+int dy_stem_pipelined(const float* img_nchw, int w);
 int dy_stem_forward(const float* img_nchw, const float* weight, void* raw, int ldraw, double* acc, int n, int h, int w, float mul,
                     hipStream_t stream);
 int dy_stem_forward_eval(const float* img_nchw, const float* weight, const float* bias, void* y, int ldy, int n, int h, int w, float mul,
```

Measured after the change: 6135 images/s, median of 6. 1.2% higher.
